# luuk666/Lightweight-MASt3R-SLAM

Hardware: AMD Instinct MI355X
Metric: tracked frames/s (match+GN, 512x512 pointmaps) @1 GPU; BA edges/s @1/2/4/8 (higher is better)
Workload: dtype f32 (refine f16, GN accum f64); 1 GPU; TUM fr1_room tracking-only, config/calib.yaml (calib mode), 512x512 pointmap pairs, GN to convergence; parallelism=replicas x1 (tracking does not shard), ring_pairs=6

## Files before the change

lightweight-mast3r-slam_amd/csrc/abi_match.cpp:

```cpp
#include "abi_common.h"
#include "m3s_match.h"

using namespace m3s_abi;

extern "C" int m3s_iter_proj(const float* rays, const float* pts, const float* p_init, float* p_new,
                             uint8_t* converged, int B, int H, int W, int C, int N, int max_iter, float lambda_init,
                             float cost_thresh, void* stream) {
  M3S_CHECK(B >= 0 && N >= 0 && H >= 3 && W >= 3, "iter_proj: image must be at least 3x3");
  M3S_CHECK(C == 9, "iter_proj: rays_img_with_grad must have 9 channels (ray, gx, gy)");
  M3S_CHECK(max_iter >= 0, "iter_proj: max_iter must be >= 0");
  if (B == 0 || N == 0) return M3S_OK;
  M3S_CHECK(rays && pts && p_init && p_new && converged, "iter_proj: null pointer");
  HIP_TRY(m3s_launch_iter_proj(rays, pts, p_init, p_new, converged, B, H, W, N, max_iter, lambda_init, cost_thresh,
                               (hipStream_t)stream),
          "iter_proj launch");
  return M3S_OK;
}

extern "C" int m3s_refine_matches(int dtype, const void* D11, const void* D21, const int64_t* p1, int64_t* p1_new,
                                  int B, int H, int W, int F, int N, int radius, int dilation_max, void* stream) {
  M3S_CHECK(B >= 0 && N >= 0 && H >= 1 && W >= 1, "refine_matches: bad shape");
  M3S_CHECK(radius >= 0 && dilation_max >= 0, "refine_matches: radius/dilation_max must be >= 0");
  if (B == 0 || N == 0) return M3S_OK;
  M3S_CHECK(D11 && D21 && p1 && p1_new, "refine_matches: null pointer");
  if (dtype == 0) {
    M3S_CHECK(F == 16 || F == 24 || F == 32, "refine_matches: f16 path supports F in {16,24,32}");
    HIP_TRY(m3s_launch_refine_f16(D11, D21, p1, p1_new, B, H, W, F, N, radius, dilation_max, (hipStream_t)stream),
            "refine_matches launch");
  } else if (dtype == 1) {
    M3S_CHECK(F >= 1, "refine_matches: F must be >= 1");
    HIP_TRY(m3s_launch_refine_f32((const float*)D11, (const float*)D21, p1, p1_new, B, H, W, F, N, radius,
                                  dilation_max, (hipStream_t)stream),
            "refine_matches launch");
  } else {
    return fail(M3S_EINVAL, "refine_matches: dtype must be 0 (f16) or 1 (f32)");
  }
  return M3S_OK;
}

namespace {
struct MatchWs {
  float* rays9;
  void* D11h;
  int* p1;
  float* cpart;
  float* cmax;
};
}

static size_t match_carve(Carver& c, int B, int H, int W, int F, MatchWs* w) {
  w->rays9 = c.take<float>((size_t)B * H * W * 9);
  w->D11h = c.take<uint16_t>((size_t)B * H * W * F);
  w->p1 = c.take<int>((size_t)B * H * W * 2);
  w->cpart = c.take<float>((size_t)m3s_prep_parts(B, H, W));
  w->cmax = c.take<float>(1);
  return c.off;
}

extern "C" size_t m3s_match_workspace_size(int B, int H, int W, int F) {
  Carver c(nullptr);
  MatchWs w;
  return match_carve(c, B, H, W, F, &w);
}

extern "C" int m3s_match(const float* X11, const float* X21, const float* D11, const float* D21,
                         const int64_t* idx_init, int64_t* idx_out, uint8_t* valid_out, int B, int H, int W, int F,
                         int max_iter, float lambda_init, float cost_thresh, float dist_thresh, int radius,
                         int dilation_max, void* workspace, size_t workspace_bytes, void* stream) {
  M3S_CHECK(B >= 1 && H >= 3 && W >= 3, "match: image must be at least 3x3");
  M3S_CHECK(F == 16 || F == 24 || F == 32, "match: descriptor dim must be 16, 24 or 32");
  M3S_CHECK(X11 && X21 && D11 && D21 && idx_out && valid_out, "match: null pointer");
  M3S_CHECK(max_iter >= 0 && radius >= 0 && dilation_max >= 0, "match: negative parameter");
  if (workspace_bytes < m3s_match_workspace_size(B, H, W, F)) return fail(M3S_ESPACE, "match: workspace too small");
  Carver c(workspace);
  MatchWs w;
  match_carve(c, B, H, W, F, &w);
  hipStream_t s = (hipStream_t)stream;
  const int planar = radius > 0 && m3s_refine_tile_ok(B, H, W, F, radius, dilation_max);
  const bool screen = env_flag("M3S_REFINE_SCREEN", true) && planar;
  {
    Span sp("prep_rays", s);
    HIP_TRY(m3s_launch_prep(X11, w.rays9, radius > 0 ? D11 : nullptr, w.D11h, B, H, W, F, planar,
                            screen ? w.cpart : nullptr, s),
            "match prep launch");
  }
  const bool fuse = planar && env_flag("M3S_MATCH_FUSE_PROJ", true) && (size_t)9 * H * W < ((size_t)1 << 31);
  if (fuse) {
    Span sp("refine_lin", s);
    HIP_TRY(m3s_launch_refine_tile_proj(w.D11h, D21, idx_out, valid_out, w.rays9, X11, X21, idx_init, B, H, W, F, radius,
                                        dilation_max, max_iter, lambda_init, cost_thresh, dist_thresh,
                                        screen ? w.cpart : nullptr, m3s_prep_parts(B, H, W), s),
            "match fused proj + refine launch");
    return M3S_OK;
  }
  {
    Span sp("proj_occlusion", s);
    HIP_TRY(m3s_launch_proj_occlusion(w.rays9, X11, X21, idx_init, w.p1, valid_out, B, H, W, max_iter, lambda_init,
                                      cost_thresh, dist_thresh, w.cpart, m3s_prep_parts(B, H, W),
                                      screen ? w.cmax : nullptr, s),
            "match proj launch");
  }
  {
    Span sp("refine_lin", s);
    HIP_TRY(m3s_launch_refine_lin(w.D11h, D21, w.p1, idx_out, B, H, W, F, radius, radius > 0 ? dilation_max : 0,
                                  screen ? w.cmax : nullptr, s),
            "match refine launch");
  }
  return M3S_OK;
}
```

lightweight-mast3r-slam_amd/csrc/m3s_match.h:

```cpp
#pragma once
#include <stdint.h>
#include <hip/hip_runtime.h>

extern "C" {
hipError_t m3s_launch_prep(const float* X11, float* rays9, const float* D11, void* D11h, int B, int H, int W, int F,
                           int planar, float* cnorm_part, hipStream_t s);
int m3s_prep_parts(int B, int H, int W);
hipError_t m3s_launch_iter_proj(const float* rays, const float* pts, const float* p_init, float* p_new, uint8_t* conv,
                                int B, int H, int W, int N, int max_iter, float lambda_init, float cost_thresh,
                                hipStream_t s);
hipError_t m3s_launch_proj_occlusion(const float* rays, const float* X11, const float* X21, const int64_t* idx_init,
                                     int* p1, uint8_t* valid, int B, int H, int W, int max_iter, float lambda_init,
                                     float cost_thresh, float dist_thresh, const float* cnorm_part, int nparts,
                                     float* cmax, hipStream_t s);
hipError_t m3s_launch_refine_f16(const void* D11, const void* D21, const int64_t* p1, int64_t* p1_new, int B, int H,
                                 int W, int F, int N, int radius, int dilation_max, hipStream_t s);
hipError_t m3s_launch_refine_f32(const float* D11, const float* D21, const int64_t* p1, int64_t* p1_new, int B, int H,
                                 int W, int F, int N, int radius, int dilation_max, hipStream_t s);
hipError_t m3s_launch_refine_lin(const void* D11h, const float* D21, const int* p1, int64_t* idx_out, int B, int H,
                                 int W, int F, int radius, int dilation_max, const float* cmax, hipStream_t s);
int m3s_refine_tile_ok(int B, int H, int W, int F, int radius, int dilation_max);
hipError_t m3s_launch_refine_tile(const void* D11h, const void* D21, const void* p1, void* out, int B, int H, int W,
                                  int F, int radius, int dilation_max, int fused, const float* cmax, hipStream_t s);
hipError_t m3s_launch_refine_tile_proj(const void* D11h, const float* D21, int64_t* idx_out, uint8_t* valid,
                                       const float* rays9, const float* X11, const float* X21, const int64_t* idx_init,
                                       int B, int H, int W, int F, int radius, int dilation_max, int max_iter,
                                       float lambda_init, float cost_thresh, float dist_thresh,
                                       const float* cnorm_part, int nparts, hipStream_t s);
}
```

lightweight-mast3r-slam_amd/csrc/m3s_proj.hpp:

```cpp
#pragma once
#include "m3s_half.hpp"

namespace m3s {

__device__ __forceinline__ float norm3_ref(float x, float y, float z) {
  return sqrtf(__builtin_fmaf(z, z, __builtin_fmaf(y, y, x * x)));
}

__device__ __forceinline__ float reduce_cnorm_wave(const float* __restrict__ part, int nparts) {
  const int lane = threadIdx.x & 63;
  float m = 0.0f;
  for (int base = lane; base < nparts; base += 64 * 16) {
    float v[16];
#pragma unroll
    for (int k = 0; k < 16; k++) v[k] = part[min(base + 64 * k, nparts - 1)];
#pragma unroll
    for (int k = 0; k < 16; k++) m = fmaxf_nan(m, v[k]);
  }
#pragma unroll
  for (int off = 32; off > 0; off >>= 1) m = fmaxf_nan(m, __shfl_xor(m, off, 64));
  return m;
}

__device__ __forceinline__ void reduce_cnorm(const float* __restrict__ part, int nparts, float* __restrict__ cmax) {
  const float m = reduce_cnorm_wave(part, nparts);
  if ((threadIdx.x & 63) == 0) *cmax = m;
}

__device__ __forceinline__ void bilin_w(float u, float v, int& u11, int& v11, float w[4]) {
  u11 = (int)floorf(u);
  v11 = (int)floorf(v);
  const float du = u - (float)u11;
  const float dv = v - (float)v11;
  const float cu = 1.0f - du, cv = 1.0f - dv;
  w[0] = du * dv;
  w[1] = cu * dv;
  w[2] = du * cv;
  w[3] = cu * cv;
}

__device__ __forceinline__ void bilin_sample9(const float* __restrict__ img, int W, int u11, int v11, const float w[4],
                                              float* out) {
  typedef float wf2 __attribute__((ext_vector_type(2)));
  const unsigned o = (unsigned)(v11 * W + u11) * 9u;
  const float* r22 = img + o;
  const float* r21 = r22 + 9;
  const float* r12 = img + (o + 9u * (unsigned)W);
  const float* r11 = r12 + 9;
  const wf2 w0 = {w[0], w[0]}, w1 = {w[1], w[1]}, w2 = {w[2], w[2]}, w3 = {w[3], w[3]};
  auto ld2 = [](const float* q) {
    wf2 r;
    r.x = q[0];
    r.y = q[1];
    return r;
  };
#pragma unroll
  for (int j = 0; j < 8; j += 2) {
    const wf2 o = w0 * ld2(r11 + j) + w1 * ld2(r12 + j) + w2 * ld2(r21 + j) + w3 * ld2(r22 + j);
    out[j] = o.x;
    out[j + 1] = o.y;
  }
  out[8] = w[0] * r11[8] + w[1] * r12[8] + w[2] * r21[8] + w[3] * r22[8];
}

struct LmState {
  float u, v, lambda, cost, e0, e1, e2;
  float s[9];
  bool conv;
};

template <bool LAST>
__device__ __forceinline__ void lm_iter(LmState& m, const float* __restrict__ img, int H, int W, const float p[3],
                                        float cost_thresh, const float* __restrict__ X11b, float* xo) {
  const float* s = m.s;
  float A00 = s[3] * s[3] + s[4] * s[4] + s[5] * s[5];
  const float A01 = s[3] * s[6] + s[4] * s[7] + s[5] * s[8];
  float A11 = s[6] * s[6] + s[7] * s[7] + s[8] * s[8];
  const float b0 = -(m.e0 * s[3] + m.e1 * s[4] + m.e2 * s[5]);
  const float b1 = -(m.e0 * s[6] + m.e1 * s[7] + m.e2 * s[8]);
  A00 += m.lambda;
  A11 += m.lambda;
  const float det_inv = 1.0f / (A00 * A11 - A01 * A01);
  float u_new = m.u + det_inv * (A11 * b0 - A01 * b1);
  float v_new = m.v + det_inv * (-A01 * b0 + A00 * b1);
  u_new = fminf(fmaxf(u_new, 1.0f), (float)(W - 2));
  v_new = fminf(fmaxf(v_new, 1.0f), (float)(H - 2));
  float xa[3], xb[3];
  if constexpr (LAST) {
    const float* qa = X11b + ((size_t)(int)v_new * W + (int)u_new) * 3;
    const float* qb = X11b + ((size_t)(int)m.v * W + (int)m.u) * 3;
#pragma unroll
    for (int c = 0; c < 3; c++) {
      xa[c] = qa[c];
      xb[c] = qb[c];
    }
  }
  int u11, v11;
  float w[4], t[9];
  bilin_w(u_new, v_new, u11, v11, w);
  bilin_sample9(img, W, u11, v11, w, t);
  const float r_norm_inv = 1.0f / sqrtf(t[0] * t[0] + t[1] * t[1] + t[2] * t[2]);
  const float f0 = t[0] * r_norm_inv - p[0];
  const float f1 = t[1] * r_norm_inv - p[1];
  const float f2 = t[2] * r_norm_inv - p[2];
  const float new_cost = f0 * f0 + f1 * f1 + f2 * f2;
  if (new_cost < m.cost) {
    m.u = u_new;
    m.v = v_new;
#pragma unroll
    for (int k = 0; k < 9; k++) m.s[k] = t[k];
    m.e0 = f0;
    m.e1 = f1;
    m.e2 = f2;
    m.conv = new_cost < cost_thresh;
    m.cost = new_cost;
    m.lambda = (float)((double)m.lambda * 0.1);
    if constexpr (LAST) {
#pragma unroll
      for (int c = 0; c < 3; c++) xo[c] = xa[c];
    }
  } else {
    m.lambda = (float)((double)m.lambda * 10.0);
    m.conv = m.cost < cost_thresh;
    if constexpr (LAST) {
#pragma unroll
      for (int c = 0; c < 3; c++) xo[c] = xb[c];
    }
  }
}

template <bool OCC>
__device__ __forceinline__ void iter_proj_point(const float* __restrict__ img, int H, int W, const float p[3],
                                                float& u, float& v, bool& conv, int max_iter, float lambda_init,
                                                float cost_thresh, const float* __restrict__ X11b = nullptr,
                                                float* xo = nullptr) {
  LmState m;
  m.u = fminf(fmaxf(u, 1.0f), (float)(W - 2));
  m.v = fminf(fmaxf(v, 1.0f), (float)(H - 2));
  m.lambda = lambda_init;
  m.conv = conv;
  int u11, v11;
  float w[4];
  if constexpr (OCC) {
    if (max_iter <= 0) {
      const float* q = X11b + ((size_t)(int)m.v * W + (int)m.u) * 3;
#pragma unroll
      for (int c = 0; c < 3; c++) xo[c] = q[c];
    }
  }
  bilin_w(m.u, m.v, u11, v11, w);
  bilin_sample9(img, W, u11, v11, w, m.s);
  const float r_norm_inv = 1.0f / sqrtf(m.s[0] * m.s[0] + m.s[1] * m.s[1] + m.s[2] * m.s[2]);
  m.e0 = m.s[0] * r_norm_inv - p[0];
  m.e1 = m.s[1] * r_norm_inv - p[1];
  m.e2 = m.s[2] * r_norm_inv - p[2];
  m.cost = m.e0 * m.e0 + m.e1 * m.e1 + m.e2 * m.e2;
  if constexpr (OCC) {
    for (int i = 0; i < max_iter - 1; i++) lm_iter<false>(m, img, H, W, p, cost_thresh, nullptr, nullptr);
    if (max_iter > 0) lm_iter<true>(m, img, H, W, p, cost_thresh, X11b, xo);
  } else {
    for (int i = 0; i < max_iter; i++) lm_iter<false>(m, img, H, W, p, cost_thresh, nullptr, nullptr);
  }
  u = m.u;
  v = m.v;
  conv = m.conv;
}

__device__ __forceinline__ void lin_to_pixel_f(int64_t i0, int W, float& u, float& v) {
  if (i0 >= 0 && i0 <= 0x7fffffff) {
    const unsigned q = (unsigned)i0 / (unsigned)W;
    u = (float)((unsigned)i0 - q * (unsigned)W);
    v = (float)q;
    return;
  }
  int64_t vq = i0 / W, uq = i0 % W;
  if (uq < 0) {
    uq += W;
    vq -= 1;
  }
  u = (float)uq;
  v = (float)vq;
}

}
```

lightweight-mast3r-slam_amd/csrc/matching.hip:

```cpp
#include "m3s_proj.hpp"
#include "m3s_match.h"

namespace m3s {

__device__ __forceinline__ void desc_load(const float* __restrict__ D11, int b, int n, int N, float4 v[6]) {
  const float4* src = reinterpret_cast<const float4*>(D11 + ((size_t)b * N + min(n, N - 1)) * 24);
#pragma unroll
  for (int k = 0; k < 6; k++) v[k] = src[k];
}

__device__ __forceinline__ float desc_planar(const float4 v[6], h1* __restrict__ D11h, int b, int n, int N) {
  float ss = 0.0f;
  if (n < N) {
    const size_t plane = (size_t)N * 8;
    h1* dst = D11h + (size_t)b * 3 * plane + (size_t)n * 8;
#pragma unroll
    for (int c = 0; c < 3; c++) {
      const float4 v0 = v[2 * c], v1 = v[2 * c + 1];
      h1 r[8] = {(h1)v0.x, (h1)v0.y, (h1)v0.z, (h1)v0.w, (h1)v1.x, (h1)v1.y, (h1)v1.z, (h1)v1.w};
      *reinterpret_cast<uint4*>(dst + c * plane) = *reinterpret_cast<uint4*>(r);
#pragma unroll
      for (int k = 0; k < 8; k++) ss += (float)r[k] * (float)r[k];
    }
  }
  return ss;
}

#define PREP_T 16
template <int DMODE>
__global__ void __launch_bounds__(256) prep_rays_kernel(const float* __restrict__ X11, float* __restrict__ rays9,
                                                        const float* __restrict__ D11, h1* __restrict__ D11h, int H,
                                                        int W, int F, float* __restrict__ cnorm_part) {
  __shared__ float tile[(PREP_T + 2) * (PREP_T + 2) * 3];
  const int b = blockIdx.z;
  const int u0 = blockIdx.x * PREP_T, v0 = blockIdx.y * PREP_T;
  const float* Xb = X11 + (size_t)b * H * W * 3;
  const int lx = threadIdx.x % PREP_T, ly = threadIdx.x / PREP_T;
  const int x = u0 + lx, y = v0 + ly;
  constexpr bool planar_d = DMODE == 1;
  const int dn = (x < W && y < H) ? y * W + x : H * W;
  constexpr int HALO = (PREP_T + 2) * (PREP_T + 2);
  static_assert(HALO <= 2 * 256, "prep halo: two pixels per thread");
  float hv[2][3];
#pragma unroll
  for (int r = 0; r < 2; r++) {
    const int t = min((int)threadIdx.x + 256 * r, HALO - 1);
    const int hy = t / (PREP_T + 2), hx = t % (PREP_T + 2);
    int yy = v0 + hy - 1, xx = u0 + hx - 1;
    yy = yy < 0 ? -yy : (yy >= H ? 2 * H - 2 - yy : yy);
    xx = xx < 0 ? -xx : (xx >= W ? 2 * W - 2 - xx : xx);
    yy = min(max(yy, 0), H - 1);
    xx = min(max(xx, 0), W - 1);
    const float* p = Xb + ((size_t)yy * W + xx) * 3;
    hv[r][0] = p[0];
    hv[r][1] = p[1];
    hv[r][2] = p[2];
  }
  float4 dv[6];
  if constexpr (planar_d) desc_load(D11, b, dn, H * W, dv);
#pragma unroll
  for (int r = 0; r < 2; r++) {
    const int t = threadIdx.x + 256 * r;
    if (t < HALO) {
      const float a = hv[r][0], c = hv[r][1], d = hv[r][2];
      const float n = fmaxf(norm3_ref(a, c, d), 1e-12f);
      tile[t * 3 + 0] = a / n;
      tile[t * 3 + 1] = c / n;
      tile[t * 3 + 2] = d / n;
    }
  }
  __syncthreads();
  if (x < W && y < H) {
    float* o = rays9 + (((size_t)b * H + y) * W + x) * 9;
#define T3(dy, dx, c) tile[(((ly + 1 + (dy)) * (PREP_T + 2)) + (lx + 1 + (dx))) * 3 + (c)]
#pragma unroll
    for (int c = 0; c < 3; c++) {
      o[c] = T3(0, 0, c);
      const float t00 = T3(-1, -1, c), t01 = T3(-1, 0, c), t02 = T3(-1, 1, c), t10 = T3(0, -1, c), t11 = T3(0, 0, c),
                  t12 = T3(0, 1, c), t20 = T3(1, -1, c), t21 = T3(1, 0, c), t22 = T3(1, 1, c);
      float gx = -0.09375f * t00;
      gx = __builtin_fmaf(0.0f, t01, gx);
      gx = __builtin_fmaf(0.09375f, t02, gx);
      gx = __builtin_fmaf(-0.3125f, t10, gx);
      gx = __builtin_fmaf(0.0f, t11, gx);
      gx = __builtin_fmaf(0.3125f, t12, gx);
      gx = __builtin_fmaf(-0.09375f, t20, gx);
      gx = __builtin_fmaf(0.0f, t21, gx);
      gx = __builtin_fmaf(0.09375f, t22, gx);
      float gy = -0.09375f * t00;
      gy = __builtin_fmaf(-0.3125f, t01, gy);
      gy = __builtin_fmaf(-0.09375f, t02, gy);
      gy = __builtin_fmaf(0.0f, t10, gy);
      gy = __builtin_fmaf(0.0f, t11, gy);
      gy = __builtin_fmaf(0.0f, t12, gy);
      gy = __builtin_fmaf(0.09375f, t20, gy);
      gy = __builtin_fmaf(0.3125f, t21, gy);
      gy = __builtin_fmaf(0.09375f, t22, gy);
      o[3 + c] = gx;
      o[6 + c] = gy;
    }
#undef T3
  }
  if constexpr (planar_d) {
    const float ss = desc_planar(dv, D11h, b, dn, H * W);
    if (cnorm_part != nullptr) {
      __shared__ float s_max[4];
      float nmax = sqrtf(ss);
#pragma unroll
      for (int off = 32; off > 0; off >>= 1) nmax = fmaxf_nan(nmax, __shfl_xor(nmax, off, 64));
      if ((threadIdx.x & 63) == 0) s_max[threadIdx.x >> 6] = nmax;
      __syncthreads();
      if (threadIdx.x == 0)
        cnorm_part[((size_t)b * gridDim.y + blockIdx.y) * gridDim.x + blockIdx.x] =
            fmaxf_nan(fmaxf_nan(s_max[0], s_max[1]), fmaxf_nan(s_max[2], s_max[3]));
    }
  } else if constexpr (DMODE == 2) {
    for (int t = threadIdx.x; t < PREP_T * PREP_T * (F / 4); t += blockDim.x) {
      const int pix = t / (F / 4), q = t % (F / 4);
      const int xx = u0 + pix % PREP_T, yy = v0 + pix / PREP_T;
      if (xx < W && yy < H) {
        const size_t off = (((size_t)b * H + yy) * W + xx) * F + q * 4;
        const float4 v = *reinterpret_cast<const float4*>(D11 + off);
        h1 r[4] = {(h1)v.x, (h1)v.y, (h1)v.z, (h1)v.w};
        *reinterpret_cast<uint2*>(D11h + off) = *reinterpret_cast<uint2*>(r);
      }
    }
  }
}


__global__ void __launch_bounds__(256) iter_proj_kernel(const float* __restrict__ rays, const float* __restrict__ pts,
                                                        const float* __restrict__ p_init, float* __restrict__ p_new,
                                                        uint8_t* __restrict__ converged, int H, int W, int N,
                                                        int max_iter, float lambda_init, float cost_thresh) {
  const int n = blockIdx.x * blockDim.x + threadIdx.x;
  const int b = blockIdx.y;
  if (n >= N) return;
  const size_t bn = (size_t)b * N + n;
  const float p[3] = {pts[bn * 3 + 0], pts[bn * 3 + 1], pts[bn * 3 + 2]};
  float u = p_init[bn * 2 + 0], v = p_init[bn * 2 + 1];
  bool conv = false;
  iter_proj_point<false>(rays + (size_t)b * H * W * 9, H, W, p, u, v, conv, max_iter, lambda_init, cost_thresh);
  p_new[bn * 2 + 0] = u;
  p_new[bn * 2 + 1] = v;
  converged[bn] = conv;
}

__global__ void __launch_bounds__(256) proj_occlusion_kernel(
    const float* __restrict__ rays, const float* __restrict__ X11, const float* __restrict__ X21,
    const int64_t* __restrict__ idx_init, int* __restrict__ p1, uint8_t* __restrict__ valid, int H, int W,
    int max_iter, float lambda_init, float cost_thresh, float dist_thresh, const float* __restrict__ cnorm_part,
    int nparts, float* __restrict__ cmax) {
  const int N = H * W;
  if (cmax != nullptr && blockIdx.x == 0 && blockIdx.y == 0 && threadIdx.x < 64) reduce_cnorm(cnorm_part, nparts, cmax);
  const int n = xcd_remap(blockIdx.x, gridDim.x) * blockDim.x + threadIdx.x;
  const int b = blockIdx.y;
  if (n >= N) return;
  const size_t bn = (size_t)b * N + n;
  const float x = X21[bn * 3 + 0], y = X21[bn * 3 + 1], z = X21[bn * 3 + 2];
  const float nrm = fmaxf(norm3_ref(x, y, z), 1e-12f);
  const float p[3] = {x / nrm, y / nrm, z / nrm};
  float u, v;
  lin_to_pixel_f(idx_init != nullptr ? idx_init[bn] : (int64_t)n, W, u, v);
  bool conv = false;
  float Xg[3];
  iter_proj_point<true>(rays + (size_t)b * H * W * 9, H, W, p, u, v, conv, max_iter, lambda_init, cost_thresh,
                        X11 + (size_t)b * H * W * 3, Xg);
  const int pu = (int)u, pv = (int)v;
  const float dx = Xg[0] - x, dy = Xg[1] - y, dz = Xg[2] - z;
  const float d = norm3_ref(dx, dy, dz);
  p1[bn * 2 + 0] = pu;
  p1[bn * 2 + 1] = pv;
  valid[bn] = conv && (d < dist_thresh);
}

template <int F>
__device__ __forceinline__ h1 score_f16(const h2* q, const h1* __restrict__ c) {
  h2 cv[F / 2];
  const uint4* c4 = reinterpret_cast<const uint4*>(c);
#pragma unroll
  for (int k = 0; k < F / 8; k++) {
    const uint4 t = c4[k];
    cv[4 * k + 0] = *reinterpret_cast<const h2*>(&t.x);
    cv[4 * k + 1] = *reinterpret_cast<const h2*>(&t.y);
    cv[4 * k + 2] = *reinterpret_cast<const h2*>(&t.z);
    cv[4 * k + 3] = *reinterpret_cast<const h2*>(&t.w);
  }
  h1 s = (h1)0.0f;
#pragma unroll
  for (int k = 0; k < F / 2; k++) {
    const h2 pr = q[k] * cv[k];
    s = s + pr.x;
    s = s + pr.y;
  }
  return s;
}

template <class S, class Score>
__device__ __forceinline__ void refine_point(int H, int W, int radius, int dilation_max, S start, int& u0, int& v0,
                                             Score score) {
  S max_score = start;
  int u_new = u0, v_new = v0;
  for (int d = dilation_max; d > 0; d--) {
    const int rd = radius * d;
    const int diam = 2 * rd + 1;
    for (int i = 0; i < diam; i += d) {
      const int u = u0 - rd + i;
      for (int j = 0; j < diam; j += d) {
        const int v = v0 - rd + j;
        if (v >= 0 && v < H && u >= 0 && u < W) {
          const S s = score((size_t)v * W + u);
          if (s > max_score) {
            max_score = s;
            u_new = u;
            v_new = v;
          }
        }
      }
    }
    u0 = u_new;
    v0 = v_new;
  }
}
template <int F>
__device__ __forceinline__ void refine_point_f16(const h1* __restrict__ img, int H, int W, const h2* q, int radius,
                                                 int dilation_max, int& u0, int& v0) {
  refine_point(H, W, radius, dilation_max, (h1)0.0f, u0, v0,
               [&](size_t pix) { return score_f16<F>(q, img + pix * F); });
}

template <int F>
__global__ void __launch_bounds__(256) refine_f16_kernel(const h1* __restrict__ D11, const h1* __restrict__ D21,
                                                         const int64_t* __restrict__ p1, int64_t* __restrict__ p1_new,
                                                         int H, int W, int N, int radius, int dilation_max) {
  const int n = blockIdx.x * blockDim.x + threadIdx.x;
  const int b = blockIdx.y;
  if (n >= N) return;
  const size_t bn = (size_t)b * N + n;
  h2 q[F / 2];
  load_query<F, false>(D21, bn, q);
  int u0 = (int)p1[bn * 2 + 0], v0 = (int)p1[bn * 2 + 1];
  refine_point_f16<F>(D11 + (size_t)b * H * W * F, H, W, q, radius, dilation_max, u0, v0);
  p1_new[bn * 2 + 0] = u0;
  p1_new[bn * 2 + 1] = v0;
}

template <int F>
__global__ void __launch_bounds__(256) refine_lin_kernel(const h1* __restrict__ D11h, const float* __restrict__ D21,
                                                         const int* __restrict__ p1, int64_t* __restrict__ idx_out,
                                                         int H, int W, int radius, int dilation_max) {
  const int N = H * W;
  const int n = blockIdx.x * blockDim.x + threadIdx.x;
  const int b = blockIdx.y;
  if (n >= N) return;
  const size_t bn = (size_t)b * N + n;
  h2 q[F / 2];
  load_query<F, true>(D21, bn, q);
  int u0 = p1[bn * 2 + 0], v0 = p1[bn * 2 + 1];
  refine_point_f16<F>(D11h + (size_t)b * H * W * F, H, W, q, radius, dilation_max, u0, v0);
  idx_out[bn] = (int64_t)u0 + (int64_t)W * v0;
}

__global__ void __launch_bounds__(256) refine_f32_kernel(const float* __restrict__ D11, const float* __restrict__ D21,
                                                         const int64_t* __restrict__ p1, int64_t* __restrict__ p1_new,
                                                         int H, int W, int F, int N, int radius, int dilation_max) {
  const int n = blockIdx.x * blockDim.x + threadIdx.x;
  const int b = blockIdx.y;
  if (n >= N) return;
  const size_t bn = (size_t)b * N + n;
  const float* q = D21 + bn * F;
  const float* img = D11 + (size_t)b * H * W * F;
  int u0 = (int)p1[bn * 2 + 0], v0 = (int)p1[bn * 2 + 1];
  refine_point(H, W, radius, dilation_max, 1.17549435e-38f , u0, v0, [&](size_t pix) {
    const float* c = img + pix * F;
    float s = 0.0f;
    for (int k = 0; k < F; k++) s += q[k] * c[k];
    return s;
  });
  p1_new[bn * 2 + 0] = u0;
  p1_new[bn * 2 + 1] = v0;
}

}

extern "C" hipError_t m3s_launch_prep(const float* X11, float* rays9, const float* D11, void* D11h, int B, int H,
                                      int W, int F, int planar, float* cnorm_part, hipStream_t s) {
  dim3 grid((W + PREP_T - 1) / PREP_T, (H + PREP_T - 1) / PREP_T, B);
  auto k = D11 == nullptr ? m3s::prep_rays_kernel<0> : planar ? m3s::prep_rays_kernel<1> : m3s::prep_rays_kernel<2>;
  hipLaunchKernelGGL(k, grid, dim3(256), 0, s, X11, rays9, D11, reinterpret_cast<m3s::h1*>(D11h), H, W, F,
                     cnorm_part);
  return hipGetLastError();
}

extern "C" int m3s_prep_parts(int B, int H, int W) {
  return B * ((W + PREP_T - 1) / PREP_T) * ((H + PREP_T - 1) / PREP_T);
}

extern "C" hipError_t m3s_launch_iter_proj(const float* rays, const float* pts, const float* p_init, float* p_new,
                                           uint8_t* conv, int B, int H, int W, int N, int max_iter, float lambda_init,
                                           float cost_thresh, hipStream_t s) {
  if ((size_t)9 * H * W >= ((size_t)1 << 31)) return hipErrorInvalidValue;
  dim3 grid((N + 255) / 256, B);
  hipLaunchKernelGGL(m3s::iter_proj_kernel, grid, dim3(256), 0, s, rays, pts, p_init, p_new, conv, H, W, N,
                     max_iter, lambda_init, cost_thresh);
  return hipGetLastError();
}

extern "C" hipError_t m3s_launch_proj_occlusion(const float* rays, const float* X11, const float* X21,
                                                const int64_t* idx_init, int* p1, uint8_t* valid, int B, int H, int W,
                                                int max_iter, float lambda_init, float cost_thresh, float dist_thresh,
                                                const float* cnorm_part, int nparts, float* cmax, hipStream_t s) {
  if ((size_t)9 * H * W >= ((size_t)1 << 31)) return hipErrorInvalidValue;
  dim3 grid((H * W + 255) / 256, B);
  hipLaunchKernelGGL(m3s::proj_occlusion_kernel, grid, dim3(256), 0, s, rays, X11, X21, idx_init, p1, valid, H, W,
                     max_iter, lambda_init, cost_thresh, dist_thresh, cnorm_part, nparts, cmax);
  return hipGetLastError();
}

template <class L>
static hipError_t refine_with_F(int F, L&& launch) {
  switch (F) {
    case 16: launch(std::integral_constant<int, 16>{}); break;
    case 24: launch(std::integral_constant<int, 24>{}); break;
    case 32: launch(std::integral_constant<int, 32>{}); break;
    default: return hipErrorInvalidValue;
  }
  return hipGetLastError();
}

extern "C" hipError_t m3s_launch_refine_f16(const void* D11, const void* D21, const int64_t* p1, int64_t* p1_new, int B,
                                            int H, int W, int F, int N, int radius, int dilation_max, hipStream_t s) {
  dim3 grid((N + 255) / 256, B);
  const m3s::h1* a = reinterpret_cast<const m3s::h1*>(D11);
  const m3s::h1* q = reinterpret_cast<const m3s::h1*>(D21);
  if (N == H * W &&
      m3s_launch_refine_tile(D11, D21, p1, p1_new, B, H, W, F, radius, dilation_max, 0, nullptr, s) == hipSuccess)
    return hipSuccess;
  return refine_with_F(F, [&](auto f) {
    hipLaunchKernelGGL(m3s::refine_f16_kernel<decltype(f)::value>, grid, dim3(256), 0, s, a, q, p1, p1_new, H, W, N,
                       radius, dilation_max);
  });
}

extern "C" hipError_t m3s_launch_refine_f32(const float* D11, const float* D21, const int64_t* p1, int64_t* p1_new,
                                            int B, int H, int W, int F, int N, int radius, int dilation_max,
                                            hipStream_t s) {
  dim3 grid((N + 255) / 256, B);
  hipLaunchKernelGGL(m3s::refine_f32_kernel, grid, dim3(256), 0, s, D11, D21, p1, p1_new, H, W, F, N, radius,
                     dilation_max);
  return hipGetLastError();
}

extern "C" hipError_t m3s_launch_refine_lin(const void* D11h, const float* D21, const int* p1, int64_t* idx_out, int B,
                                            int H, int W, int F, int radius, int dilation_max, const float* cmax,
                                            hipStream_t s) {
  dim3 grid((H * W + 255) / 256, B);
  const m3s::h1* a = reinterpret_cast<const m3s::h1*>(D11h);
  if (radius > 0 && m3s_refine_tile_ok(B, H, W, F, radius, dilation_max))
    return m3s_launch_refine_tile(D11h, D21, p1, idx_out, B, H, W, F, radius, dilation_max, 1, cmax, s);
  return refine_with_F(F, [&](auto f) {
    hipLaunchKernelGGL(m3s::refine_lin_kernel<decltype(f)::value>, grid, dim3(256), 0, s, a, D21, p1, idx_out, H, W,
                       radius, dilation_max);
  });
}
```

lightweight-mast3r-slam_amd/csrc/refine.hip:

```cpp
#include "m3s_proj.hpp"
#include "m3s_match.h"

namespace m3s {

constexpr int RT_TW = 32, RT_TH = 8, RT_WAVES = 4, RT_THREADS = 64 * RT_WAVES;
constexpr int RT_MIN_BLOCKS = 16 / RT_WAVES;
constexpr int RT_ROWS = 40, RT_COLS = 64;
constexpr int RT_PROWS = 17, RT_PCOLS = 48, RT_PPLANE = RT_PROWS * RT_PCOLS;
constexpr int RT_DROWS = 26, RT_DBUF = RT_DROWS * RT_PCOLS;
static_assert(RT_TH == 2 * RT_WAVES, "two pixel rows per wave");
static_assert(3 * RT_PROWS * RT_PCOLS <= RT_ROWS * RT_COLS && 2 * RT_DROWS * RT_PCOLS <= RT_ROWS * RT_COLS,
              "the packed and double-buffered windows share the block's window");

typedef __attribute__((address_space(1))) const void* gvoid_t;
typedef __attribute__((address_space(3))) void* lvoid_t;

constexpr int RT_PRIO_LM = 3, RT_PRIO_START = 3, RT_PRIO_FILL = 3, RT_PRIO_SURV = 3, RT_PRIO_SCORE = 2,
              RT_PRIO_LAG = 1;
constexpr int rt_prio_at(int p, int d) {
  const int q = (RT_PRIO_LAG && d > 0 && d < 3) ? p - (3 - d) : p;
  return q < 0 ? 0 : (q > 3 ? 3 : q);
}
template <int P, int D = 0>
__device__ __forceinline__ void rt_prio() {
  __builtin_amdgcn_s_setprio(rt_prio_at(P, D));
}
template <int FROM, int P, int D>
__device__ __forceinline__ void rt_prio_from() {
  if constexpr (rt_prio_at(FROM, D) != rt_prio_at(P, D)) __builtin_amdgcn_s_setprio(rt_prio_at(P, D));
}

#ifdef M3S_REFINE_STATS
__device__ unsigned long long g_refine_stats[64];
#endif
template <int D>
__device__ __forceinline__ void stats_outliers(int lane, uint64_t om) {
#ifdef M3S_REFINE_STATS
  if (lane == 0 && om) {
    atomicAdd(&g_refine_stats[2 * D], (unsigned long long)__popcll(om));
    atomicAdd(&g_refine_stats[2 * D + 1], 1ull);
  }
#endif
}
template <int D>
__device__ __forceinline__ void stats_survivors(int lane, uint64_t m) {
#ifdef M3S_REFINE_STATS
  int mx = __popcll(m), sm = mx;
#pragma unroll
  for (int off = 32; off > 0; off >>= 1) {
    mx = max(mx, __shfl_xor(mx, off, 64));
    sm += __shfl_xor(sm, off, 64);
  }
  if (lane == __ffsll((long long)__ballot(1)) - 1) {
    atomicAdd(&g_refine_stats[32 + 2 * D], (unsigned long long)sm);
    atomicAdd(&g_refine_stats[33 + 2 * D], (unsigned long long)mx);
  }
#endif
}
#ifdef M3S_REFINE_BSTAMPS
__device__ unsigned long long g_refine_bstamps[8192 * 4];
#endif
__device__ __forceinline__ unsigned long long bstamp_clock() {
#ifdef M3S_REFINE_BSTAMPS
  return __builtin_amdgcn_s_memrealtime();
#else
  return 0ull;
#endif
}
__device__ __forceinline__ void bstamp_levels_start(bool fuse_proj, unsigned long long stamp_top) {
#ifdef M3S_REFINE_BSTAMPS
  if (threadIdx.x == 0 && blockIdx.x < 8192)
    g_refine_bstamps[blockIdx.x * 4 + 0] = fuse_proj ? stamp_top : __builtin_amdgcn_s_memrealtime();
#endif
}
__device__ __forceinline__ void bstamp_block_end(bool fuse_proj, unsigned long long stamp_lm, bool active,
                                                 uint4* lds) {
#ifdef M3S_REFINE_BSTAMPS
  const unsigned long long nact = __popcll(__ballot(active));
  unsigned long long* s_act = reinterpret_cast<unsigned long long*>(&lds[0]);
  __syncthreads();
  if ((threadIdx.x & 63) == 0) s_act[threadIdx.x >> 6] = nact;
  __syncthreads();
  if (threadIdx.x == 0 && blockIdx.x < 8192) {
    unsigned hw;
    asm volatile("s_getreg_b32 %0, hwreg(HW_REG_HW_ID)" : "=s"(hw));
    g_refine_bstamps[blockIdx.x * 4 + 1] = __builtin_amdgcn_s_memrealtime();
    g_refine_bstamps[blockIdx.x * 4 + 2] = hw;
    unsigned long long na = 0;
    for (int w = 0; w < RT_WAVES; w++) na += s_act[w];
    g_refine_bstamps[blockIdx.x * 4 + 3] = fuse_proj ? stamp_lm : na;
  }
#endif
}

template <bool PLANAR>
__device__ __forceinline__ const h1* pix_ptr(const h1* img, size_t pix) {
  return img + pix * (PLANAR ? 8 : 24);
}
template <bool PLANAR>
__device__ __forceinline__ void load_chunks(const h1* p, size_t N, uint4& c0, uint4& c1, uint4& c2) {
  const size_t cs = PLANAR ? N * 8 : 8;
  c0 = *reinterpret_cast<const uint4*>(p);
  c1 = *reinterpret_cast<const uint4*>(p + cs);
  c2 = *reinterpret_cast<const uint4*>(p + 2 * cs);
}

__device__ __forceinline__ h1 exact_score(const h2* q, uint4 c0, uint4 c1, uint4 c2) {
  h1 sc = (h1)0.0f;
  add8(sc, &q[0], c0);
  add8(sc, &q[4], c1);
  add8(sc, &q[8], c2);
  return sc;
}
__device__ __forceinline__ void take_if_greater(h1 sc, int c, h1& max_score, int& bi) {
  if (sc > max_score) {
    max_score = sc;
    bi = c;
  }
}

template <int D, bool PLANAR>
__device__ __forceinline__ void wave_level(const h1* __restrict__ img, int H, int W, const h2* sq, int& cu, int& cv,
                                           h1& max_score, int lane) {
  constexpr int R = 3, RD = R * D, G = 2 * R + 1;
  const int ci = lane / G, cj = lane % G;
  const int u = cu - RD + ci * D, v = cv - RD + cj * D;
  const bool ok = lane < G * G && u >= 0 && u < W && v >= 0 && v < H;
  uint4 c0, c1, c2;
  load_chunks<PLANAR>(pix_ptr<PLANAR>(img, (size_t)min(max(v, 0), H - 1) * W + min(max(u, 0), W - 1)),
                      (size_t)H * W, c0, c1, c2);
  const h1 sc = exact_score(sq, c0, c1, c2);
  const float sf = (ok && sc == sc) ? (float)sc : -INFINITY;
  float vmax = sf;
#pragma unroll
  for (int off = 32; off > 0; off >>= 1) vmax = fmaxf(vmax, __shfl_xor(vmax, off, 64));
  const int first = __ffsll((long long)__ballot(sf == vmax)) - 1;
  if (vmax > (float)max_score) {
    max_score = (h1)vmax;
    cu = cu - RD + (first / G) * D;
    cv = cv - RD + (first % G) * D;
  }
}

template <int D>
__device__ __forceinline__ void score_chunk(const uint4* base, const h2* q4, h1* s) {
  constexpr int G = 7;
#pragma unroll
  for (int i = 0; i < G; i++) {
#pragma unroll
    for (int j = 0; j < G; j++) add8(s[i * G + j], q4, base[j * D * RT_COLS + i * D]);
    __builtin_amdgcn_sched_barrier(0);
  }
}

template <int D, int STRIDE = RT_COLS>
__device__ __forceinline__ void screen_chunk(const uint4* base, const h2* q4, float* a, bool seed = false) {
  constexpr int G = 7;
#pragma unroll
  for (int i = 0; i < G; i++) {
    uint4 c[G];
#pragma unroll
    for (int j = 0; j < G; j++) c[j] = base[j * D * STRIDE + i * D];
#pragma unroll
    for (int j = 0; j < G; j++) {
      const h2* cv = reinterpret_cast<const h2*>(&c[j]);
      float t = seed ? 0.0f : a[i * G + j];
#pragma unroll
      for (int k = 0; k < 4; k++) t = __builtin_amdgcn_fdot2(q4[k], cv[k], t, false);
      a[i * G + j] = t;
    }
    float* ac = &a[i * G];
    asm volatile("" : "+v"(ac[0]), "+v"(ac[1]), "+v"(ac[2]), "+v"(ac[3]), "+v"(ac[4]), "+v"(ac[5]), "+v"(ac[6]));
    __builtin_amdgcn_sched_barrier(0);
  }
}

__device__ __forceinline__ uint64_t screen_mask(const float* a, float T) {
  constexpr int C = 49;
  unsigned lo = 0u, hi = 0u;
  unsigned long long s[C];
#pragma unroll
  for (int k = 0; k < C + 2; k++) {
    if (k < C) asm volatile("v_cmp_ge_f32_e64 %0, %1, %2" : "=s"(s[k]) : "v"(a[C - 1 - k]), "v"(T));
    if (k >= 2) {
      unsigned long long co;
      if (C - 1 - (k - 2) >= 32)
        asm volatile("v_addc_co_u32_e64 %0, %1, %0, %0, %2" : "+v"(hi), "=s"(co) : "s"(s[k - 2]));
      else
        asm volatile("v_addc_co_u32_e64 %0, %1, %0, %0, %2" : "+v"(lo), "=s"(co) : "s"(s[k - 2]));
    }
  }
  return ((uint64_t)hi << 32) | lo;
}

template <int D, bool PLANAR>
__device__ __forceinline__ void exact_survivors(const h1* __restrict__ img, int H, int W, const h2* q, int u_lo,
                                                int v_lo, uint64_t m, h1& max_score, int& bi) {
  while (__ballot(m != 0)) {
    int c[2];
    uint4 x[2][3];
#pragma unroll
    for (int k = 0; k < 2; k++) {
      c[k] = m != 0 ? __ffsll((long long)m) - 1 : -1;
      m &= m - 1;
    }
    rt_prio_from<RT_PRIO_SCORE, RT_PRIO_SURV, D>();
#pragma unroll
    for (int k = 0; k < 2; k++) {
      if (c[k] >= 0) {
        const int i = c[k] / 7, j = c[k] - 7 * i;
        load_chunks<PLANAR>(pix_ptr<PLANAR>(img, (size_t)(v_lo + j * D) * W + (u_lo + i * D)), (size_t)H * W, x[k][0],
                            x[k][1], x[k][2]);
      }
    }
    rt_prio_from<RT_PRIO_SURV, RT_PRIO_SCORE, D>();
#pragma unroll
    for (int k = 0; k < 2; k++)
      if (c[k] >= 0) take_if_greater(exact_score(q, x[k][0], x[k][1], x[k][2]), c[k], max_score, bi);
  }
}

__device__ __forceinline__ void lds_dma_row(const h1* g, unsigned lds_addr) {
  const unsigned m0 = __builtin_amdgcn_readfirstlane(lds_addr);
  asm volatile("s_nop 0\n\tglobal_load_lds_dwordx4 %0, off" ::"v"(g), "{m0}"(m0) : "memory");
}

template <int D>
__device__ __forceinline__ void exact_survivors_lds(const uint4* base, const h2* q, uint64_t m, h1& max_score,
                                                    int& bi) {
  while (m != 0) {
    const int c = __ffsll((long long)m) - 1;
    m &= m - 1;
    const int i = c / 7, j = c - 7 * i;
    const uint4* p = base + j * D * RT_PCOLS + i * D;
    take_if_greater(exact_score(q, p[0], p[RT_PPLANE], p[2 * RT_PPLANE]), c, max_score, bi);
  }
}

struct TileCtx {
  const h1* img;
  int H, W, lane, wid, u_pix, v_pix;
  int fu, fv;
  int tcu, tcv;
  float bq = 0.0f;
  bool sok = false;
};

struct LevelWin {
  int wx0, wy0;
  int nrows, ncols;
  bool packed, dbuf;
  bool col_in;
  int lane_off;
};

struct LaneGrid {
  int u_lo, v_lo;
  int bx, by;
  bool in;
};
template <int D>
__device__ __forceinline__ void recentre(const LaneGrid& g, int bi, int& cu, int& cv) {
  if (bi >= 0) {
    cu = g.u_lo + (bi / 7) * D;
    cv = g.v_lo + (bi % 7) * D;
  }
}

template <bool PLANAR, bool ASM_DMA>
__device__ __forceinline__ void fill_rows(const TileCtx& t, const LevelWin& w, uint4* dst, int stride, int chunk,
                                          int y0) {
  const size_t cstride = PLANAR ? (size_t)t.H * t.W * 8 : 8, rstride = (size_t)t.W * (PLANAR ? 8 : 24);
  for (int y = y0; y < w.nrows; y += RT_WAVES) {
    const int gy = min(max(w.wy0 + y, 0), t.H - 1);
    const h1* rowp = t.img + (size_t)gy * rstride + chunk * cstride;
    if (w.col_in) {
      if constexpr (ASM_DMA)
        lds_dma_row(rowp + w.lane_off, (unsigned)(uintptr_t)(lvoid_t)&dst[y * stride]);
      else
        __builtin_amdgcn_global_load_lds((gvoid_t)(rowp + w.lane_off), (lvoid_t)&dst[y * stride], 16, 0, 0);
    }
  }
}

template <int D, bool SCREEN, bool PLANAR>
__device__ __forceinline__ LevelWin level_window(const TileCtx& t, bool active, int cu, int cv, int (*s_red)[4]) {
  constexpr int RD = 3 * D;
  const int lane = t.lane, wid = t.wid;
  const bool inl = active && abs(cu - t.u_pix - t.fu) <= 16 && abs(cv - t.v_pix - t.fv) <= 16;
  constexpr int NONE = 0x7fff7fff;
  const int pk = __builtin_bit_cast(int, __builtin_amdgcn_cvt_pk_i16(cu, cv));
  const int red = wave_reduce2(inl ? pk : NONE, inl ? ~pk : NONE, [](int a, int b) { return pk_min_i16(a, b); });
  __syncthreads();
  if ((lane & 31) == 0) s_red[wid][lane >> 5] = red;
  __syncthreads();
  int lo = s_red[0][0], hi = s_red[0][1];
#pragma unroll
  for (int w = 1; w < RT_WAVES; w++) {
    lo = pk_min_i16(lo, s_red[w][0]);
    hi = pk_min_i16(hi, s_red[w][1]);
  }
  hi = ~hi;
  int mnu = (int)(short)lo, mnv = lo >> 16, mxu = (int)(short)hi, mxv = hi >> 16;
  if (mnu > mxu) {
    mnu = mxu = 0;
    mnv = mxv = 0;
  }
  const int x_lo = mnu - RD, x_hi = mxu + RD, y_lo = mnv - RD, y_hi = mxv + RD;
  LevelWin w;
  w.packed = w.dbuf = false;
  if constexpr (SCREEN && D == 1) w.packed = x_hi - x_lo + 1 <= RT_PCOLS && y_hi - y_lo + 1 <= RT_PROWS;
  if constexpr (SCREEN && D == 2) w.dbuf = x_hi - x_lo + 1 <= RT_PCOLS && y_hi - y_lo + 1 <= RT_DROWS;
  const int wc = (w.packed || w.dbuf) ? RT_PCOLS : RT_COLS;
  const int wr = w.packed ? RT_PROWS : (w.dbuf ? RT_DROWS : RT_ROWS);
  w.wx0 = (x_hi - x_lo + 1 <= wc) ? x_lo : t.tcu - wc / 2;
  w.wy0 = (y_hi - y_lo + 1 <= wr) ? y_lo : t.tcv - wr / 2;
  w.nrows = min(wr, y_hi - w.wy0 + 1);
  w.ncols = min(wc, x_hi - w.wx0 + 1);
  w.col_in = lane < w.ncols;
  w.lane_off = min(max(w.wx0 + lane, 0), t.W - 1) * (PLANAR ? 8 : 24);
  return w;
}

template <int D, bool PLANAR>
__device__ __forceinline__ void level_outliers(const TileCtx& t, bool outl, const h2* q, int& cu, int& cv,
                                               h1& max_score) {
  constexpr int F = 24;
  const int lane = t.lane;
  uint64_t m = __ballot(outl);
  stats_outliers<D>(lane, m);
  while (m) {
    const int src = __ffsll((long long)m) - 1;
    m &= m - 1;
    int scu = __shfl(cu, src, 64), scv = __shfl(cv, src, 64);
    const unsigned short mb0 = (unsigned short)__shfl((int)*reinterpret_cast<const unsigned short*>(&max_score),
                                                      src, 64);
    h1 smax = *reinterpret_cast<const h1*>(&mb0);
    h2 sq[F / 2];
#pragma unroll
    for (int k = 0; k < F / 2; k++) {
      const int v = __shfl(*reinterpret_cast<const int*>(&q[k]), src, 64);
      sq[k] = *reinterpret_cast<const h2*>(&v);
    }
    wave_level<D, PLANAR>(t.img, t.H, t.W, sq, scu, scv, smax, lane);
    if (lane == src) {
      cu = scu;
      cv = scv;
      max_score = smax;
    }
  }
}

template <int D, bool PLANAR, class Scorer>
__device__ __forceinline__ void general_window(const TileCtx& t, const LevelWin& w, uint4* lds, bool lane_in,
                                               Scorer score) {
#pragma unroll
  for (int chunk = 0; chunk < 3; chunk++) {
    if (chunk) {
      rt_prio_from<RT_PRIO_SCORE, RT_PRIO_FILL, D>();
      __syncthreads();
    }
    fill_rows<PLANAR, false>(t, w, lds, RT_COLS, chunk, t.wid);
    asm volatile("s_waitcnt vmcnt(0)" ::: "memory");
    __syncthreads();
    rt_prio_from<RT_PRIO_FILL, RT_PRIO_SCORE, D>();
    if (lane_in) score(chunk);
  }
}

template <int D>
__device__ __forceinline__ uint64_t in_image_mask(int u_lo, int v_lo, int H, int W) {
  constexpr int G = 7;
  uint64_t jm = 0, vm = 0;
#pragma unroll
  for (int j = 0; j < G; j++) jm |= (v_lo + j * D >= 0 && v_lo + j * D < H) ? (1ull << j) : 0ull;
#pragma unroll
  for (int i = 0; i < G; i++) vm |= (u_lo + i * D >= 0 && u_lo + i * D < W) ? (jm << (i * G)) : 0ull;
  return vm;
}
template <int D>
__device__ __forceinline__ bool wave_leaves_image(const LaneGrid& g, int H, int W) {
  return __ballot(g.in && !(g.u_lo >= 0 && g.u_lo + 6 * D < W && g.v_lo >= 0 && g.v_lo + 6 * D < H)) != 0;
}

template <int D, bool PLANAR>
__device__ __forceinline__ void screened_level(const TileCtx& t, const LevelWin& w, const LaneGrid& g, const h2* q,
                                               int& cu, int& cv, h1& max_score, uint4* lds, bool first) {
  constexpr int G = 7;
  const int wid = t.wid, H = t.H, W = t.W;
  float a[G * G];
  __syncthreads();
  rt_prio_from<RT_PRIO_START, RT_PRIO_FILL, D>();
  const int b0 = g.by * RT_PCOLS + g.bx;
  if (w.packed) {
    for (int chunk = 0; chunk < 3; chunk++)
      fill_rows<PLANAR, false>(t, w, &lds[chunk * RT_PPLANE], RT_PCOLS, chunk,
                               (wid - chunk * w.nrows) & (RT_WAVES - 1));
    asm volatile("s_waitcnt vmcnt(0)" ::: "memory");
    __syncthreads();
    rt_prio_from<RT_PRIO_FILL, RT_PRIO_SCORE, D>();
    if (g.in) {
#pragma unroll
      for (int chunk = 0; chunk < 3; chunk++)
        screen_chunk<D, RT_PCOLS>(&lds[chunk * RT_PPLANE + b0], &q[chunk * 4], a, chunk == 0);
    }
  } else if (w.dbuf) {
    fill_rows<PLANAR, true>(t, w, lds, RT_PCOLS, 0, wid);
    asm volatile("s_waitcnt vmcnt(0)" ::: "memory");
    __builtin_amdgcn_s_waitcnt(0x0F70);
    __syncthreads();
#pragma unroll
    for (int chunk = 0; chunk < 3; chunk++) {
      if (chunk < 2) fill_rows<PLANAR, true>(t, w, &lds[((chunk + 1) & 1) * RT_DBUF], RT_PCOLS, chunk + 1, wid);
      rt_prio_from<RT_PRIO_FILL, RT_PRIO_SCORE, D>();
      if (g.in) screen_chunk<D, RT_PCOLS>(&lds[(chunk & 1) * RT_DBUF + b0], &q[chunk * 4], a, chunk == 0);
      if (chunk < 2) {
        rt_prio_from<RT_PRIO_SCORE, RT_PRIO_FILL, D>();
        asm volatile("s_waitcnt vmcnt(0)" ::: "memory");
        __syncthreads();
      }
    }
  } else {
    general_window<D, PLANAR>(t, w, lds, g.in, [&](int chunk) {
      screen_chunk<D>(&lds[g.by * RT_COLS + g.bx], &q[chunk * 4], a, chunk == 0);
    });
  }
  if (g.in) {
    uint64_t vm = (1ull << (G * G)) - 1ull;
    if (wave_leaves_image<D>(g, H, W)) {
      vm = in_image_mask<D>(g.u_lo, g.v_lo, H, W);
#pragma unroll
      for (int c = 0; c < G * G; c++) a[c] = ((vm >> c) & 1ull) ? a[c] : -INFINITY;
    }
    float lmax = a[0];
#pragma unroll
    for (int c = 1; c < G * G; c++)
      if (c != G * G / 2) lmax = fmaxf(lmax, a[c]);
    lmax = fmaxf(lmax, first ? a[G * G / 2] : -INFINITY);
    const float tms = (float)max_score - t.bq;
    if (__builtin_amdgcn_readfirstlane((int)(__ballot(!t.sok || lmax >= tms) != 0ull)) == 0) return;
    const float T = fmaxf(tms, lmax - 2.0f * t.bq);
    uint64_t m = screen_mask(a, T);
    if (!t.sok) m = ~0ull;
    m &= vm;
    if (!first) m &= ~(1ull << (G * G / 2));
    stats_survivors<D>(t.lane, m);
    int bi = -1;
    if (w.packed)
      exact_survivors_lds<D>(&lds[b0], q, m, max_score, bi);
    else
      exact_survivors<D, PLANAR>(t.img, H, W, q, g.u_lo, g.v_lo, m, max_score, bi);
    recentre<D>(g, bi, cu, cv);
  }
}

template <bool MASKED>
__device__ __forceinline__ void exact_scan(const h1* s, uint64_t vm, h1& max_score, int& bi) {
#pragma unroll
  for (int c = 0; c < 49; c++) {
    const bool gt = (!MASKED || ((vm >> c) & 1ull)) && s[c] > max_score;
    max_score = gt ? s[c] : max_score;
    bi = gt ? c : bi;
  }
}

template <int D, bool PLANAR>
__device__ __forceinline__ void exact_level(const TileCtx& t, const LevelWin& w, const LaneGrid& g, const h2* q,
                                            int& cu, int& cv, h1& max_score, uint4* lds) {
  constexpr int G = 7;
  h1 s[G * G];
#pragma unroll
  for (int c = 0; c < G * G; c++) s[c] = (h1)0.0f;
  __syncthreads();
  rt_prio_from<RT_PRIO_START, RT_PRIO_FILL, D>();
  general_window<D, PLANAR>(t, w, lds, g.in, [&](int chunk) {
    score_chunk<D>(&lds[g.by * RT_COLS + g.bx], &q[chunk * 4], s);
  });
  if (g.in) {
    int bi = -1;
    if (!wave_leaves_image<D>(g, t.H, t.W))
      exact_scan<false>(s, 0ull, max_score, bi);
    else
      exact_scan<true>(s, in_image_mask<D>(g.u_lo, g.v_lo, t.H, t.W), max_score, bi);
    recentre<D>(g, bi, cu, cv);
  }
}

template <int D, bool SCREEN, bool PLANAR>
__device__ __forceinline__ void refine_level(const TileCtx& t, bool active, const h2* q, int& cu, int& cv,
                                             h1& max_score, uint4* lds, int (*s_red)[4], bool first) {
  constexpr int RD = 3 * D;
  rt_prio<RT_PRIO_START, D>();
  const LevelWin w = level_window<D, SCREEN, PLANAR>(t, active, cu, cv, s_red);
  LaneGrid g;
  g.u_lo = cu - RD;
  g.v_lo = cv - RD;
  g.bx = g.u_lo - w.wx0;
  g.by = g.v_lo - w.wy0;
  g.in = active && g.bx >= 0 && g.bx + 2 * RD < w.ncols && g.by >= 0 && g.by + 2 * RD < w.nrows;
  level_outliers<D, PLANAR>(t, active && !g.in, q, cu, cv, max_score);
  if constexpr (SCREEN)
    screened_level<D, PLANAR>(t, w, g, q, cu, cv, max_score, lds, first);
  else
    exact_level<D, PLANAR>(t, w, g, q, cu, cv, max_score, lds);
}


template <bool P1_I64>
__device__ __forceinline__ void load_p1(const void* p1v, size_t bn, int& cu, int& cv) {
  if constexpr (P1_I64) {
    cu = (int)reinterpret_cast<const int64_t*>(p1v)[bn * 2];
    cv = (int)reinterpret_cast<const int64_t*>(p1v)[bn * 2 + 1];
  } else {
    cu = reinterpret_cast<const int*>(p1v)[bn * 2];
    cv = reinterpret_cast<const int*>(p1v)[bn * 2 + 1];
  }
}

template <bool LIN_OUT>
__device__ __forceinline__ void store_out(void* outv, size_t bn, int W, int cu, int cv) {
  if constexpr (LIN_OUT) {
    reinterpret_cast<int64_t*>(outv)[bn] = (int64_t)cu + (int64_t)W * cv;
  } else {
    reinterpret_cast<int64_t*>(outv)[bn * 2] = cu;
    reinterpret_cast<int64_t*>(outv)[bn * 2 + 1] = cv;
  }
}

struct ProjArgs {
  const float* rays9;
  const float* X11;
  const float* X21;
  const int64_t* idx_init;
  uint8_t* valid;
  const float* cnorm_part;
  int nparts, max_iter;
  float lambda_init, cost_thresh, dist_thresh;
};

template <bool SCREEN>
__device__ __forceinline__ void proj_prologue(const TileCtx& t, const ProjArgs& pa, const void* D21, int b,
                                              bool active, size_t bn, int& cu, int& cv, float4* dv, float& cmax_w) {
  constexpr int F = 24;
  const int H = t.H, W = t.W, N = H * W;
  rt_prio_from<0, RT_PRIO_LM, 0>();
  const int n = min(t.v_pix, H - 1) * W + min(t.u_pix, W - 1);
  const size_t bnc = (size_t)b * N + n;
  const float x = pa.X21[bnc * 3 + 0], y = pa.X21[bnc * 3 + 1], z = pa.X21[bnc * 3 + 2];
  const int64_t i0 = pa.idx_init != nullptr ? pa.idx_init[bnc] : (int64_t)n;
  if constexpr (SCREEN) {
    if (t.wid == 0) cmax_w = reduce_cnorm_wave(pa.cnorm_part, pa.nparts);
  }
  const float nrm = fmaxf(norm3_ref(x, y, z), 1e-12f);
  const float p[3] = {x / nrm, y / nrm, z / nrm};
  float u, v;
  lin_to_pixel_f(i0, W, u, v);
  bool conv = false;
  float Xg[3];
  iter_proj_point<true>(pa.rays9 + (size_t)b * N * 9, H, W, p, u, v, conv, pa.max_iter, pa.lambda_init,
                        pa.cost_thresh, pa.X11 + (size_t)b * N * 3, Xg);
  const float4* qsrc = reinterpret_cast<const float4*>(reinterpret_cast<const float*>(D21) + bnc * F);
#pragma unroll
  for (int k = 0; k < F / 4; k++) dv[k] = qsrc[k];
  cu = (int)u;
  cv = (int)v;
  const float dx = Xg[0] - x, dy = Xg[1] - y, dz = Xg[2] - z;
  const float d = norm3_ref(dx, dy, dz);
  const uint8_t vbyte = conv && (d < pa.dist_thresh);
  if (active) pa.valid[bn] = vbyte;
}

template <bool XCHG_CMAX>
__device__ __forceinline__ float tile_flow(TileCtx& t, bool active, int cu, int cv, int tx, int ty, float cmax_w,
                                           int (*s_red)[4]) {
  float cmax_b = 0.0f;
  const int sum = wave_reduce2(active ? cu - t.u_pix : 0, active ? cv - t.v_pix : 0, [](int a, int b) { return a + b; });
  const int na = __popcll(__ballot(active));
  if ((t.lane & 31) == 0) s_red[t.wid][t.lane >> 5] = sum;
  if (t.lane == 0) {
    s_red[t.wid][2] = na;
    if constexpr (XCHG_CMAX) s_red[t.wid][3] = __float_as_int(cmax_w);
  }
  __syncthreads();
  if constexpr (XCHG_CMAX) cmax_b = __int_as_float(__builtin_amdgcn_readfirstlane(s_red[0][3]));
  int tu = 0, tv = 0, tn = 0;
#pragma unroll
  for (int w = 0; w < RT_WAVES; w++) {
    tu += s_red[w][0];
    tv += s_red[w][1];
    tn += s_red[w][2];
  }
  const int nall = max(1, tn);
  t.fu = __builtin_amdgcn_readfirstlane(tu / nall);
  t.fv = __builtin_amdgcn_readfirstlane(tv / nall);
  t.tcu = tx * RT_TW + RT_TW / 2 + t.fu;
  t.tcv = ty * RT_TH + RT_TH / 2 + t.fv;
  return cmax_b;
}

__device__ __forceinline__ void screen_bound(TileCtx& t, const h2* q, float cm) {
  float qq = 0.0f;
#pragma unroll
  for (int k = 0; k < 12; k++) qq = __builtin_amdgcn_fdot2(q[k], q[k], qq, false);
  const float pq = sqrtf(qq) * cm * 1.001f;
  t.sok = pq <= 16384.0f;
  t.bq = t.sok ? 0.0125f * pq + 0x1p-18f : 0.0f;
}

template <bool D21_F32, bool P1_I64, bool LIN_OUT, bool SCREEN, bool FUSE_PROJ = false>
__global__ void __launch_bounds__(RT_THREADS, RT_MIN_BLOCKS)
    refine_tile_kernel(const h1* __restrict__ D11h, const void* __restrict__ D21, const void* __restrict__ p1v,
                       void* __restrict__ outv, int H, int W, int dilation_max, int tiles_x, int tiles_per_img,
                       int nblocks, const float* __restrict__ cmaxp, const ProjArgs pa) {
  constexpr int F = 24;
  static_assert(!FUSE_PROJ || (D21_F32 && !P1_I64 && LIN_OUT), "the fused projection feeds the fused match path");
  const unsigned long long stamp_top = bstamp_clock();
  __shared__ uint4 lds[RT_ROWS * RT_COLS];
  int(*s_red)[4] = reinterpret_cast<int(*)[4]>(&lds[0]);
  const int lb = xcd_remap(blockIdx.x, nblocks);
  const int b = lb / tiles_per_img, tt = lb % tiles_per_img;
  const int tx = tt % tiles_x, ty = tt / tiles_x;
  TileCtx t;
  t.H = H;
  t.W = W;
  t.lane = threadIdx.x & 63;
  t.wid = threadIdx.x >> 6;
  {
    const int l = t.lane & 31;
    const int g = (l < 4 || (l >= 12 && l < 16) || (l >= 20 && l < 28)) ? 0 : 1;
    const int r = g == 0 ? (l < 4 ? l : l < 16 ? l - 8 : l - 12) : (l < 12 ? l - 4 : l < 20 ? l - 8 : l - 16);
    t.u_pix = tx * RT_TW + g * 16 + r;
    t.v_pix = ty * RT_TH + 2 * t.wid + (t.lane >> 5);
  }
  const bool active = t.u_pix < W && t.v_pix < H;
  const int N = H * W;
  const size_t bn = (size_t)b * N + (size_t)t.v_pix * W + t.u_pix;
  t.img = D11h + (size_t)b * N * F;
  h2 q[F / 2];
  int cu = 0, cv = 0;
  float4 dv[F / 4];
  float cmax_w = 0.0f;
  if constexpr (FUSE_PROJ) {
    proj_prologue<SCREEN>(t, pa, D21, b, active, bn, cu, cv, dv, cmax_w);
  } else if (active) {
    load_query<F, D21_F32>(D21, bn, q);
    load_p1<P1_I64>(p1v, bn, cu, cv);
  } else {
#pragma unroll
    for (int k = 0; k < F / 2; k++) q[k] = h2{(h1)0.0f, (h1)0.0f};
  }
  const unsigned long long stamp_lm = bstamp_clock();
  const float cmax_b = tile_flow<FUSE_PROJ && SCREEN>(t, active, cu, cv, tx, ty, cmax_w, s_red);
  if constexpr (FUSE_PROJ) {
#pragma unroll
    for (int k = 0; k < F / 4; k++) {
      q[2 * k + 0] = h2{(h1)dv[k].x, (h1)dv[k].y};
      q[2 * k + 1] = h2{(h1)dv[k].z, (h1)dv[k].w};
    }
  }
  if constexpr (SCREEN) screen_bound(t, q, FUSE_PROJ ? cmax_b : *cmaxp);
  bstamp_levels_start(FUSE_PROJ, stamp_top);
  h1 max_score = (h1)0.0f;
#define RT_LEVEL(DD)                                                                                        \
  if (dilation_max >= DD)                                                                                   \
    refine_level<DD, SCREEN, LIN_OUT>(t, active, q, cu, cv, max_score, lds, s_red, dilation_max == DD);
  RT_LEVEL(8)
  RT_LEVEL(7)
  RT_LEVEL(6)
  RT_LEVEL(5)
  RT_LEVEL(4)
  RT_LEVEL(3)
  RT_LEVEL(2)
  RT_LEVEL(1)
#undef RT_LEVEL
  rt_prio<0>();
  if (active) store_out<LIN_OUT>(outv, bn, W, cu, cv);
  bstamp_block_end(FUSE_PROJ, stamp_lm, active, lds);
}

template <bool D21_F32, bool P1_I64, bool LIN_OUT, bool SCREEN, bool FUSE_PROJ>
static void launch_tile(const void* D11h, const void* D21, const void* p1, void* out, int B, int H, int W,
                        int dilation_max, const float* cmax, const ProjArgs& pa, hipStream_t s) {
  const int tx = (W + RT_TW - 1) / RT_TW, ty = (H + RT_TH - 1) / RT_TH, nb = tx * ty * B;
  hipLaunchKernelGGL((refine_tile_kernel<D21_F32, P1_I64, LIN_OUT, SCREEN, FUSE_PROJ>), dim3(nb), dim3(RT_THREADS), 0,
                     s, reinterpret_cast<const h1*>(D11h), D21, p1, out, H, W, dilation_max, tx, tx * ty, nb, cmax, pa);
}

}

extern "C" int m3s_refine_tile_ok(int B, int H, int W, int F, int radius, int dilation_max) {
  if (F != 24 || radius != 3 || dilation_max < 1 || dilation_max > 8) return 0;
  if ((long long)B * H * W >= (1ll << 31) || H >= 32768 || W >= 32768) return 0;
  return 1;
}

extern "C" hipError_t m3s_launch_refine_tile(const void* D11h, const void* D21, const void* p1, void* out, int B,
                                             int H, int W, int F, int radius, int dilation_max, int fused,
                                             const float* cmax, hipStream_t s) {
  if (!m3s_refine_tile_ok(B, H, W, F, radius, dilation_max)) return hipErrorNotSupported;
  const m3s::ProjArgs none{};
  if (fused && cmax != nullptr)
    m3s::launch_tile<true, false, true, true, false>(D11h, D21, p1, out, B, H, W, dilation_max, cmax, none, s);
  else if (fused)
    m3s::launch_tile<true, false, true, false, false>(D11h, D21, p1, out, B, H, W, dilation_max, nullptr, none, s);
  else
    m3s::launch_tile<false, true, false, false, false>(D11h, D21, p1, out, B, H, W, dilation_max, nullptr, none, s);
  return hipGetLastError();
}

extern "C" hipError_t m3s_launch_refine_tile_proj(const void* D11h, const float* D21, int64_t* idx_out, uint8_t* valid,
                                                  const float* rays9, const float* X11, const float* X21,
                                                  const int64_t* idx_init, int B, int H, int W, int F, int radius,
                                                  int dilation_max, int max_iter, float lambda_init, float cost_thresh,
                                                  float dist_thresh, const float* cnorm_part, int nparts,
                                                  hipStream_t s) {
  if (!m3s_refine_tile_ok(B, H, W, F, radius, dilation_max)) return hipErrorNotSupported;
  if ((size_t)9 * H * W >= ((size_t)1 << 31)) return hipErrorNotSupported;
  const m3s::ProjArgs pa{rays9, X11, X21, idx_init, valid, cnorm_part, nparts, max_iter, lambda_init, cost_thresh,
                         dist_thresh};
  if (cnorm_part != nullptr)
    m3s::launch_tile<true, false, true, true, true>(D11h, D21, nullptr, idx_out, B, H, W, dilation_max, nullptr, pa, s);
  else
    m3s::launch_tile<true, false, true, false, true>(D11h, D21, nullptr, idx_out, B, H, W, dilation_max, nullptr, pa,
                                                     s);
  return hipGetLastError();
}

#ifdef M3S_REFINE_BSTAMPS
extern "C" int m3s_debug_refine_bstamps(unsigned long long* out) {
  (void)hipDeviceSynchronize();
  return hipMemcpyFromSymbol(out, HIP_SYMBOL(m3s::g_refine_bstamps), sizeof(unsigned long long) * 8192 * 4) == hipSuccess
             ? 0 : -1;
}
#endif
#ifdef M3S_REFINE_STATS
extern "C" int m3s_debug_refine_stats(unsigned long long* out, int reset) {
  (void)hipDeviceSynchronize();
  if (hipMemcpyFromSymbol(out, HIP_SYMBOL(m3s::g_refine_stats), sizeof(unsigned long long) * 64) != hipSuccess) return -1;
  if (reset) {
    unsigned long long z[64] = {0};
    (void)hipMemcpyToSymbol(HIP_SYMBOL(m3s::g_refine_stats), z, sizeof(z));
  }
  return 0;
}
#endif
```

Before: 6866 tracked frames/s.

## Add int8 descriptor screening pass to prune refine candidates before f16 scoring

The prep kernel now also quantizes reference descriptors to int8 in a side buffer and records per-block max-abs and L1 partials. The refine tile kernel uses these, with a cheap int8 bound (screen_bound8), to rule out candidate windows at dilation levels of two and above before the f16 scoring. The aim is to skip redundant f16 dot-product work in the local match refinement. In exchange it adds extra writes and bandwidth in prep, a wider cnorm reduction, and risk in the bound's correctness and in shared-memory pressure.

```diff
diff --git a/lightweight-mast3r-slam_amd/csrc/abi_match.cpp b/lightweight-mast3r-slam_amd/csrc/abi_match.cpp
--- a/lightweight-mast3r-slam_amd/csrc/abi_match.cpp
+++ b/lightweight-mast3r-slam_amd/csrc/abi_match.cpp
@@ -45,6 +45,7 @@
   int* p1;
   float* cpart;
   float* cmax;
+  void* D8;
 };
 }
 
@@ -52,8 +53,9 @@
   w->rays9 = c.take<float>((size_t)B * H * W * 9);
   w->D11h = c.take<uint16_t>((size_t)B * H * W * F);
   w->p1 = c.take<int>((size_t)B * H * W * 2);
-  w->cpart = c.take<float>((size_t)m3s_prep_parts(B, H, W));
-  w->cmax = c.take<float>(1);
+  w->cpart = c.take<float>((size_t)3 * m3s_prep_parts(B, H, W));
+  w->cmax = c.take<float>(3);
+  w->D8 = c.take<uint8_t>((size_t)B * H * W * 24 + 16);
   return c.off;
 }
 
@@ -78,10 +80,12 @@
   hipStream_t s = (hipStream_t)stream;
   const int planar = radius > 0 && m3s_refine_tile_ok(B, H, W, F, radius, dilation_max);
   const bool screen = env_flag("M3S_REFINE_SCREEN", true) && planar;
+  const bool screen8 = screen && F == 24 && env_flag("M3S_REFINE_SCREEN8", true);
+  void* const D8 = screen8 ? w.D8 : nullptr;
   {
     Span sp("prep_rays", s);
     HIP_TRY(m3s_launch_prep(X11, w.rays9, radius > 0 ? D11 : nullptr, w.D11h, B, H, W, F, planar,
-                            screen ? w.cpart : nullptr, s),
+                            screen ? w.cpart : nullptr, D8, s),
             "match prep launch");
   }
   const bool fuse = planar && env_flag("M3S_MATCH_FUSE_PROJ", true) && (size_t)9 * H * W < ((size_t)1 << 31);
@@ -89,7 +93,7 @@
     Span sp("refine_lin", s);
     HIP_TRY(m3s_launch_refine_tile_proj(w.D11h, D21, idx_out, valid_out, w.rays9, X11, X21, idx_init, B, H, W, F, radius,
                                         dilation_max, max_iter, lambda_init, cost_thresh, dist_thresh,
-                                        screen ? w.cpart : nullptr, m3s_prep_parts(B, H, W), s),
+                                        screen ? w.cpart : nullptr, m3s_prep_parts(B, H, W), D8, s),
             "match fused proj + refine launch");
     return M3S_OK;
   }
@@ -97,13 +101,13 @@
     Span sp("proj_occlusion", s);
     HIP_TRY(m3s_launch_proj_occlusion(w.rays9, X11, X21, idx_init, w.p1, valid_out, B, H, W, max_iter, lambda_init,
                                       cost_thresh, dist_thresh, w.cpart, m3s_prep_parts(B, H, W),
-                                      screen ? w.cmax : nullptr, s),
+                                      screen ? w.cmax : nullptr, screen8 ? 3 : 1, s),
             "match proj launch");
   }
   {
     Span sp("refine_lin", s);
     HIP_TRY(m3s_launch_refine_lin(w.D11h, D21, w.p1, idx_out, B, H, W, F, radius, radius > 0 ? dilation_max : 0,
-                                  screen ? w.cmax : nullptr, s),
+                                  screen ? w.cmax : nullptr, D8, s),
             "match refine launch");
   }
   return M3S_OK;
diff --git a/lightweight-mast3r-slam_amd/csrc/m3s_match.h b/lightweight-mast3r-slam_amd/csrc/m3s_match.h
--- a/lightweight-mast3r-slam_amd/csrc/m3s_match.h
+++ b/lightweight-mast3r-slam_amd/csrc/m3s_match.h
@@ -4,7 +4,7 @@
 
 extern "C" {
 hipError_t m3s_launch_prep(const float* X11, float* rays9, const float* D11, void* D11h, int B, int H, int W, int F,
-                           int planar, float* cnorm_part, hipStream_t s);
+                           int planar, float* cnorm_part, void* D8, hipStream_t s);
 int m3s_prep_parts(int B, int H, int W);
 hipError_t m3s_launch_iter_proj(const float* rays, const float* pts, const float* p_init, float* p_new, uint8_t* conv,
                                 int B, int H, int W, int N, int max_iter, float lambda_init, float cost_thresh,
@@ -12,19 +12,21 @@
 hipError_t m3s_launch_proj_occlusion(const float* rays, const float* X11, const float* X21, const int64_t* idx_init,
                                      int* p1, uint8_t* valid, int B, int H, int W, int max_iter, float lambda_init,
                                      float cost_thresh, float dist_thresh, const float* cnorm_part, int nparts,
-                                     float* cmax, hipStream_t s);
+                                     float* cmax, int nruns, hipStream_t s);
 hipError_t m3s_launch_refine_f16(const void* D11, const void* D21, const int64_t* p1, int64_t* p1_new, int B, int H,
                                  int W, int F, int N, int radius, int dilation_max, hipStream_t s);
 hipError_t m3s_launch_refine_f32(const float* D11, const float* D21, const int64_t* p1, int64_t* p1_new, int B, int H,
                                  int W, int F, int N, int radius, int dilation_max, hipStream_t s);
 hipError_t m3s_launch_refine_lin(const void* D11h, const float* D21, const int* p1, int64_t* idx_out, int B, int H,
-                                 int W, int F, int radius, int dilation_max, const float* cmax, hipStream_t s);
+                                 int W, int F, int radius, int dilation_max, const float* cmax, const void* D8,
+                                 hipStream_t s);
 int m3s_refine_tile_ok(int B, int H, int W, int F, int radius, int dilation_max);
 hipError_t m3s_launch_refine_tile(const void* D11h, const void* D21, const void* p1, void* out, int B, int H, int W,
-                                  int F, int radius, int dilation_max, int fused, const float* cmax, hipStream_t s);
+                                  int F, int radius, int dilation_max, int fused, const float* cmax, const void* D8,
+                                  hipStream_t s);
 hipError_t m3s_launch_refine_tile_proj(const void* D11h, const float* D21, int64_t* idx_out, uint8_t* valid,
                                        const float* rays9, const float* X11, const float* X21, const int64_t* idx_init,
                                        int B, int H, int W, int F, int radius, int dilation_max, int max_iter,
                                        float lambda_init, float cost_thresh, float dist_thresh,
-                                       const float* cnorm_part, int nparts, hipStream_t s);
+                                       const float* cnorm_part, int nparts, const void* D8, hipStream_t s);
 }
diff --git a/lightweight-mast3r-slam_amd/csrc/m3s_proj.hpp b/lightweight-mast3r-slam_amd/csrc/m3s_proj.hpp
--- a/lightweight-mast3r-slam_amd/csrc/m3s_proj.hpp
+++ b/lightweight-mast3r-slam_amd/csrc/m3s_proj.hpp
@@ -20,6 +20,26 @@
 #pragma unroll
   for (int off = 32; off > 0; off >>= 1) m = fmaxf_nan(m, __shfl_xor(m, off, 64));
   return m;
+}
+
+__device__ __forceinline__ void reduce_cnorm3_wave(const float* __restrict__ part, int nparts, float m[3]) {
+  const int lane = threadIdx.x & 63;
+  m[0] = m[1] = m[2] = 0.0f;
+  for (int base = lane; base < nparts; base += 64 * 16) {
+    float v[3][16];
+#pragma unroll
+    for (int r = 0; r < 3; r++)
+#pragma unroll
+      for (int k = 0; k < 16; k++) v[r][k] = part[(size_t)r * nparts + min(base + 64 * k, nparts - 1)];
+#pragma unroll
+    for (int r = 0; r < 3; r++)
+#pragma unroll
+      for (int k = 0; k < 16; k++) m[r] = fmaxf_nan(m[r], v[r][k]);
+  }
+#pragma unroll
+  for (int r = 0; r < 3; r++)
+#pragma unroll
+    for (int off = 32; off > 0; off >>= 1) m[r] = fmaxf_nan(m[r], __shfl_xor(m[r], off, 64));
 }
 
 __device__ __forceinline__ void reduce_cnorm(const float* __restrict__ part, int nparts, float* __restrict__ cmax) {
diff --git a/lightweight-mast3r-slam_amd/csrc/matching.hip b/lightweight-mast3r-slam_amd/csrc/matching.hip
--- a/lightweight-mast3r-slam_amd/csrc/matching.hip
+++ b/lightweight-mast3r-slam_amd/csrc/matching.hip
@@ -9,11 +9,15 @@
   for (int k = 0; k < 6; k++) v[k] = src[k];
 }
 
-__device__ __forceinline__ float desc_planar(const float4 v[6], h1* __restrict__ D11h, int b, int n, int N) {
+template <bool Q8>
+__device__ __forceinline__ float desc_planar(const float4 v[6], h1* __restrict__ D11h, signed char* __restrict__ D8,
+                                             int b, int n, int N, float& amax, float& c1) {
   float ss = 0.0f;
+  amax = c1 = 0.0f;
   if (n < N) {
     const size_t plane = (size_t)N * 8;
     h1* dst = D11h + (size_t)b * 3 * plane + (size_t)n * 8;
+    unsigned w8[6];
 #pragma unroll
     for (int c = 0; c < 3; c++) {
       const float4 v0 = v[2 * c], v1 = v[2 * c + 1];
@@ -21,6 +25,22 @@
       *reinterpret_cast<uint4*>(dst + c * plane) = *reinterpret_cast<uint4*>(r);
 #pragma unroll
       for (int k = 0; k < 8; k++) ss += (float)r[k] * (float)r[k];
+      if constexpr (Q8) {
+        w8[2 * c] = w8[2 * c + 1] = 0u;
+#pragma unroll
+        for (int k = 0; k < 8; k++) {
+          const float x = (float)r[k];
+          amax = fmaxf_nan(amax, fabsf(x));
+          c1 += fabsf(x);
+          const int qi = (int)rintf(fminf(fmaxf(127.0f * x, -127.0f), 127.0f));
+          w8[2 * c + (k >> 2)] |= (unsigned)(qi & 0xff) << (8 * (k & 3));
+        }
+      }
+    }
+    if constexpr (Q8) {
+      signed char* d8 = D8 + (size_t)b * N * 24;
+      *reinterpret_cast<uint4*>(d8 + (size_t)n * 16) = uint4{w8[0], w8[1], w8[2], w8[3]};
+      *reinterpret_cast<uint2*>(d8 + (size_t)N * 16 + (size_t)n * 8) = uint2{w8[4], w8[5]};
     }
   }
   return ss;
@@ -30,14 +50,15 @@
 template <int DMODE>
 __global__ void __launch_bounds__(256) prep_rays_kernel(const float* __restrict__ X11, float* __restrict__ rays9,
                                                         const float* __restrict__ D11, h1* __restrict__ D11h, int H,
-                                                        int W, int F, float* __restrict__ cnorm_part) {
+                                                        int W, int F, float* __restrict__ cnorm_part,
+                                                        signed char* __restrict__ D8) {
   __shared__ float tile[(PREP_T + 2) * (PREP_T + 2) * 3];
   const int b = blockIdx.z;
   const int u0 = blockIdx.x * PREP_T, v0 = blockIdx.y * PREP_T;
   const float* Xb = X11 + (size_t)b * H * W * 3;
   const int lx = threadIdx.x % PREP_T, ly = threadIdx.x / PREP_T;
   const int x = u0 + lx, y = v0 + ly;
-  constexpr bool planar_d = DMODE == 1;
+  constexpr bool planar_d = DMODE == 1 || DMODE == 3, q8 = DMODE == 3;
   const int dn = (x < W && y < H) ? y * W + x : H * W;
   constexpr int HALO = (PREP_T + 2) * (PREP_T + 2);
   static_assert(HALO <= 2 * 256, "prep halo: two pixels per thread");
@@ -102,17 +123,25 @@
 #undef T3
   }
   if constexpr (planar_d) {
-    const float ss = desc_planar(dv, D11h, b, dn, H * W);
+    float amax, c1;
+    const float ss = desc_planar<q8>(dv, D11h, D8, b, dn, H * W, amax, c1);
     if (cnorm_part != nullptr) {
-      __shared__ float s_max[4];
-      float nmax = sqrtf(ss);
-#pragma unroll
-      for (int off = 32; off > 0; off >>= 1) nmax = fmaxf_nan(nmax, __shfl_xor(nmax, off, 64));
-      if ((threadIdx.x & 63) == 0) s_max[threadIdx.x >> 6] = nmax;
+      constexpr int NP = q8 ? 3 : 1;
+      __shared__ float s_max[NP][4];
+      float pm[3] = {sqrtf(ss), amax, c1};
+#pragma unroll
+      for (int p = 0; p < NP; p++) {
+#pragma unroll
+        for (int off = 32; off > 0; off >>= 1) pm[p] = fmaxf_nan(pm[p], __shfl_xor(pm[p], off, 64));
+        if ((threadIdx.x & 63) == 0) s_max[p][threadIdx.x >> 6] = pm[p];
+      }
       __syncthreads();
-      if (threadIdx.x == 0)
-        cnorm_part[((size_t)b * gridDim.y + blockIdx.y) * gridDim.x + blockIdx.x] =
-            fmaxf_nan(fmaxf_nan(s_max[0], s_max[1]), fmaxf_nan(s_max[2], s_max[3]));
+      if (threadIdx.x < NP) {
+        const int p = threadIdx.x;
+        const size_t nparts = (size_t)gridDim.x * gridDim.y * gridDim.z;
+        cnorm_part[p * nparts + ((size_t)b * gridDim.y + blockIdx.y) * gridDim.x + blockIdx.x] =
+            fmaxf_nan(fmaxf_nan(s_max[p][0], s_max[p][1]), fmaxf_nan(s_max[p][2], s_max[p][3]));
+      }
     }
   } else if constexpr (DMODE == 2) {
     for (int t = threadIdx.x; t < PREP_T * PREP_T * (F / 4); t += blockDim.x) {
@@ -150,9 +179,10 @@
     const float* __restrict__ rays, const float* __restrict__ X11, const float* __restrict__ X21,
     const int64_t* __restrict__ idx_init, int* __restrict__ p1, uint8_t* __restrict__ valid, int H, int W,
     int max_iter, float lambda_init, float cost_thresh, float dist_thresh, const float* __restrict__ cnorm_part,
-    int nparts, float* __restrict__ cmax) {
+    int nparts, float* __restrict__ cmax, int nruns) {
   const int N = H * W;
-  if (cmax != nullptr && blockIdx.x == 0 && blockIdx.y == 0 && threadIdx.x < 64) reduce_cnorm(cnorm_part, nparts, cmax);
+  if (cmax != nullptr && blockIdx.x == 0 && blockIdx.y == 0 && threadIdx.x < 64)
+    for (int r = 0; r < nruns; r++) reduce_cnorm(cnorm_part + (size_t)r * nparts, nparts, cmax + r);
   const int n = xcd_remap(blockIdx.x, gridDim.x) * blockDim.x + threadIdx.x;
   const int b = blockIdx.y;
   if (n >= N) return;
@@ -284,11 +314,13 @@
 }
 
 extern "C" hipError_t m3s_launch_prep(const float* X11, float* rays9, const float* D11, void* D11h, int B, int H,
-                                      int W, int F, int planar, float* cnorm_part, hipStream_t s) {
+                                      int W, int F, int planar, float* cnorm_part, void* D8, hipStream_t s) {
   dim3 grid((W + PREP_T - 1) / PREP_T, (H + PREP_T - 1) / PREP_T, B);
-  auto k = D11 == nullptr ? m3s::prep_rays_kernel<0> : planar ? m3s::prep_rays_kernel<1> : m3s::prep_rays_kernel<2>;
+  auto k = D11 == nullptr ? m3s::prep_rays_kernel<0>
+           : !planar      ? m3s::prep_rays_kernel<2>
+           : (D8 != nullptr && cnorm_part != nullptr) ? m3s::prep_rays_kernel<3> : m3s::prep_rays_kernel<1>;
   hipLaunchKernelGGL(k, grid, dim3(256), 0, s, X11, rays9, D11, reinterpret_cast<m3s::h1*>(D11h), H, W, F,
-                     cnorm_part);
+                     cnorm_part, reinterpret_cast<signed char*>(D8));
   return hipGetLastError();
 }
 
@@ -309,11 +341,12 @@
 extern "C" hipError_t m3s_launch_proj_occlusion(const float* rays, const float* X11, const float* X21,
                                                 const int64_t* idx_init, int* p1, uint8_t* valid, int B, int H, int W,
                                                 int max_iter, float lambda_init, float cost_thresh, float dist_thresh,
-                                                const float* cnorm_part, int nparts, float* cmax, hipStream_t s) {
+                                                const float* cnorm_part, int nparts, float* cmax, int nruns,
+                                                hipStream_t s) {
   if ((size_t)9 * H * W >= ((size_t)1 << 31)) return hipErrorInvalidValue;
   dim3 grid((H * W + 255) / 256, B);
   hipLaunchKernelGGL(m3s::proj_occlusion_kernel, grid, dim3(256), 0, s, rays, X11, X21, idx_init, p1, valid, H, W,
-                     max_iter, lambda_init, cost_thresh, dist_thresh, cnorm_part, nparts, cmax);
+                     max_iter, lambda_init, cost_thresh, dist_thresh, cnorm_part, nparts, cmax, nruns);
   return hipGetLastError();
 }
 
@@ -334,7 +367,8 @@
   const m3s::h1* a = reinterpret_cast<const m3s::h1*>(D11);
   const m3s::h1* q = reinterpret_cast<const m3s::h1*>(D21);
   if (N == H * W &&
-      m3s_launch_refine_tile(D11, D21, p1, p1_new, B, H, W, F, radius, dilation_max, 0, nullptr, s) == hipSuccess)
+      m3s_launch_refine_tile(D11, D21, p1, p1_new, B, H, W, F, radius, dilation_max, 0, nullptr, nullptr, s) ==
+          hipSuccess)
     return hipSuccess;
   return refine_with_F(F, [&](auto f) {
     hipLaunchKernelGGL(m3s::refine_f16_kernel<decltype(f)::value>, grid, dim3(256), 0, s, a, q, p1, p1_new, H, W, N,
@@ -353,11 +387,11 @@
 
 extern "C" hipError_t m3s_launch_refine_lin(const void* D11h, const float* D21, const int* p1, int64_t* idx_out, int B,
                                             int H, int W, int F, int radius, int dilation_max, const float* cmax,
-                                            hipStream_t s) {
+                                            const void* D8, hipStream_t s) {
   dim3 grid((H * W + 255) / 256, B);
   const m3s::h1* a = reinterpret_cast<const m3s::h1*>(D11h);
   if (radius > 0 && m3s_refine_tile_ok(B, H, W, F, radius, dilation_max))
-    return m3s_launch_refine_tile(D11h, D21, p1, idx_out, B, H, W, F, radius, dilation_max, 1, cmax, s);
+    return m3s_launch_refine_tile(D11h, D21, p1, idx_out, B, H, W, F, radius, dilation_max, 1, cmax, D8, s);
   return refine_with_F(F, [&](auto f) {
     hipLaunchKernelGGL(m3s::refine_lin_kernel<decltype(f)::value>, grid, dim3(256), 0, s, a, D21, p1, idx_out, H, W,
                        radius, dilation_max);
diff --git a/lightweight-mast3r-slam_amd/csrc/refine.hip b/lightweight-mast3r-slam_amd/csrc/refine.hip
--- a/lightweight-mast3r-slam_amd/csrc/refine.hip
+++ b/lightweight-mast3r-slam_amd/csrc/refine.hip
@@ -8,7 +8,13 @@
 constexpr int RT_ROWS = 40, RT_COLS = 64;
 constexpr int RT_PROWS = 17, RT_PCOLS = 48, RT_PPLANE = RT_PROWS * RT_PCOLS;
 constexpr int RT_DROWS = 26, RT_DBUF = RT_DROWS * RT_PCOLS;
+constexpr int RT_8ROWS = 30, RT_8COLS = 56;
+#ifndef RT_S8_DMIN
+#define RT_S8_DMIN 2
+#endif
 static_assert(RT_TH == 2 * RT_WAVES, "two pixel rows per wave");
+static_assert(RT_8ROWS * RT_8COLS * 24 <= RT_ROWS * RT_COLS * 16, "the one-fill int8 window shares the block's window");
+static_assert(RT_8COLS % 2 == 0 && RT_8COLS <= 64 && RT_COLS == 64, "8-byte cells are filled in pairs, two rows per DMA");
 static_assert(3 * RT_PROWS * RT_PCOLS <= RT_ROWS * RT_COLS && 2 * RT_DROWS * RT_PCOLS <= RT_ROWS * RT_COLS,
               "the packed and double-buffered windows share the block's window");
 
@@ -244,12 +250,18 @@
   int tcu, tcv;
   float bq = 0.0f;
   bool sok = false;
+  const signed char* img8 = nullptr;
+  bool s8 = false;
+  bool sok8 = false;
+  float b8 = 0.0f;
+  unsigned q8[6];
 };
 
 struct LevelWin {
   int wx0, wy0;
   int nrows, ncols;
   bool packed, dbuf;
+  bool one8;
   bool col_in;
   int lane_off;
 };
@@ -308,11 +320,14 @@
   }
   const int x_lo = mnu - RD, x_hi = mxu + RD, y_lo = mnv - RD, y_hi = mxv + RD;
   LevelWin w;
-  w.packed = w.dbuf = false;
+  w.packed = w.dbuf = w.one8 = false;
+  if constexpr (SCREEN && PLANAR && D >= RT_S8_DMIN)
+    w.one8 = t.s8 && x_hi - x_lo + 1 <= RT_8COLS && y_hi - y_lo + 1 <= RT_8ROWS;
   if constexpr (SCREEN && D == 1) w.packed = x_hi - x_lo + 1 <= RT_PCOLS && y_hi - y_lo + 1 <= RT_PROWS;
-  if constexpr (SCREEN && D == 2) w.dbuf = x_hi - x_lo + 1 <= RT_PCOLS && y_hi - y_lo + 1 <= RT_DROWS;
-  const int wc = (w.packed || w.dbuf) ? RT_PCOLS : RT_COLS;
-  const int wr = w.packed ? RT_PROWS : (w.dbuf ? RT_DROWS : RT_ROWS);
+  if constexpr (SCREEN && D == 2)
+    w.dbuf = !(PLANAR && D >= RT_S8_DMIN && t.s8) && x_hi - x_lo + 1 <= RT_PCOLS && y_hi - y_lo + 1 <= RT_DROWS;
+  const int wc = (w.packed || w.dbuf) ? RT_PCOLS : (w.one8 ? RT_8COLS : RT_COLS);
+  const int wr = w.packed ? RT_PROWS : (w.dbuf ? RT_DROWS : (w.one8 ? RT_8ROWS : RT_ROWS));
   w.wx0 = (x_hi - x_lo + 1 <= wc) ? x_lo : t.tcu - wc / 2;
   w.wy0 = (y_hi - y_lo + 1 <= wr) ? y_lo : t.tcv - wr / 2;
   w.nrows = min(wr, y_hi - w.wy0 + 1);
@@ -454,6 +469,156 @@
   }
 }
 
+constexpr float RT_K8 = 127.0f * 127.0f;
+__device__ __forceinline__ int floor_i32(float x) { return (int)floorf(fminf(fmaxf(x, -2.0e9f), 2.0e9f)); }
+
+__device__ __forceinline__ void screen_bound8(TileCtx& t, const h2* q, float amax, float c1max) {
+  t.s8 = t.img8 != nullptr && amax <= 1.0f;
+  float qa = 0.0f;
+  int qn1 = 0;
+#pragma unroll
+  for (int k = 0; k < 6; k++) t.q8[k] = 0u;
+#pragma unroll
+  for (int k = 0; k < 24; k++) {
+    const float x = (k & 1) ? (float)q[k >> 1].y : (float)q[k >> 1].x;
+    qa = fmaxf_nan(qa, fabsf(x));
+    const int qi = (int)rintf(fminf(fmaxf(127.0f * x, -127.0f), 127.0f));
+    qn1 += abs(qi);
+    t.q8[k >> 2] |= (unsigned)(qi & 0xff) << (8 * (k & 3));
+  }
+  t.sok8 = t.sok && qa <= 1.0f;
+  t.b8 = t.bq + (0.5f / 127.0f) * (c1max + (float)qn1 * (1.0f / 127.0f)) * 1.001f;
+}
+
+template <int STRIDE>
+__device__ __forceinline__ void fill_rows8(const TileCtx& t, const LevelWin& w, uint4* dstA, uint4* dstB, int yA,
+                                           int yB) {
+  constexpr int LPR = STRIDE / 2;
+  const size_t N = (size_t)t.H * t.W;
+  if (dstA != nullptr) {
+    for (int y = yA; y < w.nrows; y += RT_WAVES) {
+      const int gy = min(max(w.wy0 + y, 0), t.H - 1);
+      const signed char* rowp = t.img8 + (size_t)gy * t.W * 16;
+      if (w.col_in)
+        __builtin_amdgcn_global_load_lds((gvoid_t)(rowp + 2 * w.lane_off), (lvoid_t)&dstA[y * STRIDE], 16, 0, 0);
+    }
+  }
+  if (dstB != nullptr) {
+    const int h = t.lane / LPR, l = t.lane - h * LPR;
+    const int cc = min(max(w.wx0 + 2 * l, -1), t.W - 1);
+    const bool on = h < 2 && 2 * l < w.ncols;
+    const signed char* pB = t.img8 + N * 16;
+    for (int y = yB; y < w.nrows; y += 2 * RT_WAVES) {
+      const int gy = min(max(w.wy0 + y + h, 0), t.H - 1);
+      const signed char* src = pB + ((ptrdiff_t)gy * t.W + cc) * 8;
+      if (on && y + h < w.nrows)
+        __builtin_amdgcn_global_load_lds((gvoid_t)src, (lvoid_t)&dstB[y * LPR], 16, 0, 0);
+    }
+  }
+}
+
+template <int D, int STRIDE, int NW>
+__device__ __forceinline__ void screen8_chunk(const void* basev, const unsigned* q8, int* a) {
+  constexpr int G = 7;
+  typedef typename std::conditional<NW == 4, uint4, uint2>::type V;
+  const V* base = reinterpret_cast<const V*>(basev);
+#pragma unroll
+  for (int i = 0; i < G; i++) {
+    V c[G];
+#pragma unroll
+    for (int j = 0; j < G; j++) c[j] = base[j * D * STRIDE + i * D];
+#pragma unroll
+    for (int j = 0; j < G; j++) {
+      const unsigned* cw = reinterpret_cast<const unsigned*>(&c[j]);
+      int s = NW == 4 ? 0 : a[i * G + j];
+#pragma unroll
+      for (int k = 0; k < NW; k++) s = __builtin_amdgcn_sdot4((int)q8[k], (int)cw[k], s, false);
+      a[i * G + j] = s;
+    }
+    int* ac = &a[i * G];
+    asm volatile("" : "+v"(ac[0]), "+v"(ac[1]), "+v"(ac[2]), "+v"(ac[3]), "+v"(ac[4]), "+v"(ac[5]), "+v"(ac[6]));
+    __builtin_amdgcn_sched_barrier(0);
+  }
+}
+
+__device__ __forceinline__ uint64_t screen_mask8(const int* a, int T) {
+  constexpr int C = 49;
+  unsigned lo = 0u, hi = 0u;
+  unsigned long long s[C];
+#pragma unroll
+  for (int k = 0; k < C + 2; k++) {
+    if (k < C) asm volatile("v_cmp_ge_i32_e64 %0, %1, %2" : "=s"(s[k]) : "v"(a[C - 1 - k]), "v"(T));
+    if (k >= 2) {
+      unsigned long long co;
+      if (C - 1 - (k - 2) >= 32)
+        asm volatile("v_addc_co_u32_e64 %0, %1, %0, %0, %2" : "+v"(hi), "=s"(co) : "s"(s[k - 2]));
+      else
+        asm volatile("v_addc_co_u32_e64 %0, %1, %0, %0, %2" : "+v"(lo), "=s"(co) : "s"(s[k - 2]));
+    }
+  }
+  return ((uint64_t)hi << 32) | lo;
+}
+
+template <int D, bool PLANAR>
+__device__ __forceinline__ void screened_level8(const TileCtx& t, const LevelWin& w, const LaneGrid& g, const h2* q,
+                                                int& cu, int& cv, h1& max_score, uint4* lds, bool first) {
+  constexpr int G = 7;
+  const int wid = t.wid, H = t.H, W = t.W;
+  int a[G * G];
+  __syncthreads();
+  rt_prio_from<RT_PRIO_START, RT_PRIO_FILL, D>();
+  if (w.one8) {
+    uint4* ldsB = &lds[RT_8ROWS * RT_8COLS];
+    fill_rows8<RT_8COLS>(t, w, lds, ldsB, wid, 2 * ((wid - w.nrows) & (RT_WAVES - 1)));
+    asm volatile("s_waitcnt vmcnt(0)" ::: "memory");
+    __syncthreads();
+    rt_prio_from<RT_PRIO_FILL, RT_PRIO_SCORE, D>();
+    if (g.in) {
+      const int b0 = g.by * RT_8COLS + g.bx;
+      screen8_chunk<D, RT_8COLS, 4>(&lds[b0], &t.q8[0], a);
+      screen8_chunk<D, RT_8COLS, 2>(reinterpret_cast<const uint2*>(ldsB) + b0, &t.q8[4], a);
+    }
+  } else {
+    const int b0 = g.by * RT_COLS + g.bx;
+    fill_rows8<RT_COLS>(t, w, lds, nullptr, wid, 0);
+    asm volatile("s_waitcnt vmcnt(0)" ::: "memory");
+    __syncthreads();
+    rt_prio_from<RT_PRIO_FILL, RT_PRIO_SCORE, D>();
+    if (g.in) screen8_chunk<D, RT_COLS, 4>(&lds[b0], &t.q8[0], a);
+    rt_prio_from<RT_PRIO_SCORE, RT_PRIO_FILL, D>();
+    __syncthreads();
+    fill_rows8<RT_COLS>(t, w, nullptr, lds, 0, 2 * wid);
+    asm volatile("s_waitcnt vmcnt(0)" ::: "memory");
+    __syncthreads();
+    rt_prio_from<RT_PRIO_FILL, RT_PRIO_SCORE, D>();
+    if (g.in) screen8_chunk<D, RT_COLS, 2>(reinterpret_cast<const uint2*>(lds) + b0, &t.q8[4], a);
+  }
+  if (g.in) {
+    uint64_t vm = (1ull << (G * G)) - 1ull;
+    if (wave_leaves_image<D>(g, H, W)) {
+      vm = in_image_mask<D>(g.u_lo, g.v_lo, H, W);
+#pragma unroll
+      for (int c = 0; c < G * G; c++) a[c] = ((vm >> c) & 1ull) ? a[c] : INT_MIN;
+    }
+    int lmax = a[0];
+#pragma unroll
+    for (int c = 1; c < G * G; c++)
+      if (c != G * G / 2) lmax = max(lmax, a[c]);
+    lmax = max(lmax, first ? a[G * G / 2] : INT_MIN);
+    const int tms = floor_i32(((float)max_score - t.b8) * RT_K8) - 1;
+    if (__builtin_amdgcn_readfirstlane((int)(__ballot(!t.sok8 || lmax >= tms) != 0ull)) == 0) return;
+    const int T = max(tms, floor_i32((float)lmax - 2.0f * t.b8 * RT_K8) - 1);
+    uint64_t m = screen_mask8(a, T);
+    if (!t.sok8) m = ~0ull;
+    m &= vm;
+    if (!first) m &= ~(1ull << (G * G / 2));
+    stats_survivors<D>(t.lane, m);
+    int bi = -1;
+    exact_survivors<D, PLANAR>(t.img, H, W, q, g.u_lo, g.v_lo, m, max_score, bi);
+    recentre<D>(g, bi, cu, cv);
+  }
+}
+
 template <bool MASKED>
 __device__ __forceinline__ void exact_scan(const h1* s, uint64_t vm, h1& max_score, int& bi) {
 #pragma unroll
@@ -499,7 +664,12 @@
   g.by = g.v_lo - w.wy0;
   g.in = active && g.bx >= 0 && g.bx + 2 * RD < w.ncols && g.by >= 0 && g.by + 2 * RD < w.nrows;
   level_outliers<D, PLANAR>(t, active && !g.in, q, cu, cv, max_score);
-  if constexpr (SCREEN)
+  if constexpr (SCREEN && PLANAR && D >= RT_S8_DMIN) {
+    if (t.s8)
+      screened_level8<D, PLANAR>(t, w, g, q, cu, cv, max_score, lds, first);
+    else
+      screened_level<D, PLANAR>(t, w, g, q, cu, cv, max_score, lds, first);
+  } else if constexpr (SCREEN)
     screened_level<D, PLANAR>(t, w, g, q, cu, cv, max_score, lds, first);
   else
     exact_level<D, PLANAR>(t, w, g, q, cu, cv, max_score, lds);
@@ -540,7 +710,7 @@
 
 template <bool SCREEN>
 __device__ __forceinline__ void proj_prologue(const TileCtx& t, const ProjArgs& pa, const void* D21, int b,
-                                              bool active, size_t bn, int& cu, int& cv, float4* dv, float& cmax_w) {
+                                              bool active, size_t bn, int& cu, int& cv, float4* dv, float* cmax_w) {
   constexpr int F = 24;
   const int H = t.H, W = t.W, N = H * W;
   rt_prio_from<0, RT_PRIO_LM, 0>();
@@ -549,7 +719,12 @@
   const float x = pa.X21[bnc * 3 + 0], y = pa.X21[bnc * 3 + 1], z = pa.X21[bnc * 3 + 2];
   const int64_t i0 = pa.idx_init != nullptr ? pa.idx_init[bnc] : (int64_t)n;
   if constexpr (SCREEN) {
-    if (t.wid == 0) cmax_w = reduce_cnorm_wave(pa.cnorm_part, pa.nparts);
+    if (t.wid == 0) {
+      if (t.img8 != nullptr)
+        reduce_cnorm3_wave(pa.cnorm_part, pa.nparts, cmax_w);
+      else
+        cmax_w[0] = reduce_cnorm_wave(pa.cnorm_part, pa.nparts);
+    }
   }
   const float nrm = fmaxf(norm3_ref(x, y, z), 1e-12f);
   const float p[3] = {x / nrm, y / nrm, z / nrm};
@@ -571,18 +746,25 @@
 }
 
 template <bool XCHG_CMAX>
-__device__ __forceinline__ float tile_flow(TileCtx& t, bool active, int cu, int cv, int tx, int ty, float cmax_w,
-                                           int (*s_red)[4]) {
-  float cmax_b = 0.0f;
+__device__ __forceinline__ void tile_flow(TileCtx& t, bool active, int cu, int cv, int tx, int ty,
+                                          const float* cmax_w, float* cmax_b, int (*s_red)[4]) {
   const int sum = wave_reduce2(active ? cu - t.u_pix : 0, active ? cv - t.v_pix : 0, [](int a, int b) { return a + b; });
   const int na = __popcll(__ballot(active));
   if ((t.lane & 31) == 0) s_red[t.wid][t.lane >> 5] = sum;
   if (t.lane == 0) {
     s_red[t.wid][2] = na;
-    if constexpr (XCHG_CMAX) s_red[t.wid][3] = __float_as_int(cmax_w);
+    if constexpr (XCHG_CMAX) {
+      if (t.wid == 0) {
+#pragma unroll
+        for (int r = 0; r < 3; r++) s_red[r][3] = __float_as_int(cmax_w[r]);
+      }
+    }
   }
   __syncthreads();
-  if constexpr (XCHG_CMAX) cmax_b = __int_as_float(__builtin_amdgcn_readfirstlane(s_red[0][3]));
+  if constexpr (XCHG_CMAX) {
+#pragma unroll
+    for (int r = 0; r < 3; r++) cmax_b[r] = __int_as_float(__builtin_amdgcn_readfirstlane(s_red[r][3]));
+  }
   int tu = 0, tv = 0, tn = 0;
 #pragma unroll
   for (int w = 0; w < RT_WAVES; w++) {
@@ -595,7 +777,6 @@
   t.fv = __builtin_amdgcn_readfirstlane(tv / nall);
   t.tcu = tx * RT_TW + RT_TW / 2 + t.fu;
   t.tcv = ty * RT_TH + RT_TH / 2 + t.fv;
-  return cmax_b;
 }
 
 __device__ __forceinline__ void screen_bound(TileCtx& t, const h2* q, float cm) {
@@ -611,7 +792,8 @@
 __global__ void __launch_bounds__(RT_THREADS, RT_MIN_BLOCKS)
     refine_tile_kernel(const h1* __restrict__ D11h, const void* __restrict__ D21, const void* __restrict__ p1v,
                        void* __restrict__ outv, int H, int W, int dilation_max, int tiles_x, int tiles_per_img,
-                       int nblocks, const float* __restrict__ cmaxp, const ProjArgs pa) {
+                       int nblocks, const float* __restrict__ cmaxp, const signed char* __restrict__ D8,
+                       const ProjArgs pa) {
   constexpr int F = 24;
   static_assert(!FUSE_PROJ || (D21_F32 && !P1_I64 && LIN_OUT), "the fused projection feeds the fused match path");
   const unsigned long long stamp_top = bstamp_clock();
@@ -636,10 +818,11 @@
   const int N = H * W;
   const size_t bn = (size_t)b * N + (size_t)t.v_pix * W + t.u_pix;
   t.img = D11h + (size_t)b * N * F;
+  if constexpr (SCREEN && LIN_OUT) t.img8 = D8 != nullptr ? D8 + (size_t)b * N * F : nullptr;
   h2 q[F / 2];
   int cu = 0, cv = 0;
   float4 dv[F / 4];
-  float cmax_w = 0.0f;
+  float cmax_w[3] = {0.0f, 0.0f, 0.0f}, cmax_b[3] = {0.0f, 0.0f, 0.0f};
   if constexpr (FUSE_PROJ) {
     proj_prologue<SCREEN>(t, pa, D21, b, active, bn, cu, cv, dv, cmax_w);
   } else if (active) {
@@ -650,7 +833,7 @@
     for (int k = 0; k < F / 2; k++) q[k] = h2{(h1)0.0f, (h1)0.0f};
   }
   const unsigned long long stamp_lm = bstamp_clock();
-  const float cmax_b = tile_flow<FUSE_PROJ && SCREEN>(t, active, cu, cv, tx, ty, cmax_w, s_red);
+  tile_flow<FUSE_PROJ && SCREEN>(t, active, cu, cv, tx, ty, cmax_w, cmax_b, s_red);
   if constexpr (FUSE_PROJ) {
 #pragma unroll
     for (int k = 0; k < F / 4; k++) {
@@ -658,7 +841,13 @@
       q[2 * k + 1] = h2{(h1)dv[k].z, (h1)dv[k].w};
     }
   }
-  if constexpr (SCREEN) screen_bound(t, q, FUSE_PROJ ? cmax_b : *cmaxp);
+  if constexpr (SCREEN) {
+    screen_bound(t, q, FUSE_PROJ ? cmax_b[0] : cmaxp[0]);
+    if constexpr (LIN_OUT) {
+      if (t.img8 != nullptr && dilation_max >= RT_S8_DMIN)
+        screen_bound8(t, q, FUSE_PROJ ? cmax_b[1] : cmaxp[1], FUSE_PROJ ? cmax_b[2] : cmaxp[2]);
+    }
+  }
   bstamp_levels_start(FUSE_PROJ, stamp_top);
   h1 max_score = (h1)0.0f;
 #define RT_LEVEL(DD)                                                                                        \
@@ -680,10 +869,11 @@
 
 template <bool D21_F32, bool P1_I64, bool LIN_OUT, bool SCREEN, bool FUSE_PROJ>
 static void launch_tile(const void* D11h, const void* D21, const void* p1, void* out, int B, int H, int W,
-                        int dilation_max, const float* cmax, const ProjArgs& pa, hipStream_t s) {
+                        int dilation_max, const float* cmax, const void* D8, const ProjArgs& pa, hipStream_t s) {
   const int tx = (W + RT_TW - 1) / RT_TW, ty = (H + RT_TH - 1) / RT_TH, nb = tx * ty * B;
   hipLaunchKernelGGL((refine_tile_kernel<D21_F32, P1_I64, LIN_OUT, SCREEN, FUSE_PROJ>), dim3(nb), dim3(RT_THREADS), 0,
-                     s, reinterpret_cast<const h1*>(D11h), D21, p1, out, H, W, dilation_max, tx, tx * ty, nb, cmax, pa);
+                     s, reinterpret_cast<const h1*>(D11h), D21, p1, out, H, W, dilation_max, tx, tx * ty, nb, cmax,
+                     reinterpret_cast<const signed char*>(D8), pa);
 }
 
 }
@@ -696,15 +886,17 @@
 
 extern "C" hipError_t m3s_launch_refine_tile(const void* D11h, const void* D21, const void* p1, void* out, int B,
                                              int H, int W, int F, int radius, int dilation_max, int fused,
-                                             const float* cmax, hipStream_t s) {
+                                             const float* cmax, const void* D8, hipStream_t s) {
   if (!m3s_refine_tile_ok(B, H, W, F, radius, dilation_max)) return hipErrorNotSupported;
   const m3s::ProjArgs none{};
   if (fused && cmax != nullptr)
-    m3s::launch_tile<true, false, true, true, false>(D11h, D21, p1, out, B, H, W, dilation_max, cmax, none, s);
+    m3s::launch_tile<true, false, true, true, false>(D11h, D21, p1, out, B, H, W, dilation_max, cmax, D8, none, s);
   else if (fused)
-    m3s::launch_tile<true, false, true, false, false>(D11h, D21, p1, out, B, H, W, dilation_max, nullptr, none, s);
+    m3s::launch_tile<true, false, true, false, false>(D11h, D21, p1, out, B, H, W, dilation_max, nullptr, nullptr, none,
+                                                      s);
   else
-    m3s::launch_tile<false, true, false, false, false>(D11h, D21, p1, out, B, H, W, dilation_max, nullptr, none, s);
+    m3s::launch_tile<false, true, false, false, false>(D11h, D21, p1, out, B, H, W, dilation_max, nullptr, nullptr, none,
+                                                       s);
   return hipGetLastError();
 }
 
@@ -713,16 +905,17 @@
                                                   const int64_t* idx_init, int B, int H, int W, int F, int radius,
                                                   int dilation_max, int max_iter, float lambda_init, float cost_thresh,
                                                   float dist_thresh, const float* cnorm_part, int nparts,
-                                                  hipStream_t s) {
+                                                  const void* D8, hipStream_t s) {
   if (!m3s_refine_tile_ok(B, H, W, F, radius, dilation_max)) return hipErrorNotSupported;
   if ((size_t)9 * H * W >= ((size_t)1 << 31)) return hipErrorNotSupported;
   const m3s::ProjArgs pa{rays9, X11, X21, idx_init, valid, cnorm_part, nparts, max_iter, lambda_init, cost_thresh,
                          dist_thresh};
   if (cnorm_part != nullptr)
-    m3s::launch_tile<true, false, true, true, true>(D11h, D21, nullptr, idx_out, B, H, W, dilation_max, nullptr, pa, s);
+    m3s::launch_tile<true, false, true, true, true>(D11h, D21, nullptr, idx_out, B, H, W, dilation_max, nullptr, D8, pa,
+                                                    s);
   else
-    m3s::launch_tile<true, false, true, false, true>(D11h, D21, nullptr, idx_out, B, H, W, dilation_max, nullptr, pa,
-                                                     s);
+    m3s::launch_tile<true, false, true, false, true>(D11h, D21, nullptr, idx_out, B, H, W, dilation_max, nullptr, nullptr,
+                                                     pa, s);
   return hipGetLastError();
 }
 
```

New measurement: 7104 tracked frames/s (median of 6 runs). 1.03x the previous value.
